# crisprVerse/screenCounter

Measured on AMD Instinct MI355X. Metric: Mreads/s (whole node) + achieved HBM GB/s, 100M x 150bp vs 100k barcodes <=1mm, higher is better.
Workload: dtype u8; 1 GPU; config2: countSingleBarcodes 100000000 reads x 150bp, library 100000, <=1mm, use_first=True; reads_per_gpu=100000000, read_len=150, max_mismatches=1, strand=both, parallelism=read-sharded x1, inputs=resident in HBM, settle_steps=440

## Files before the change

screencounter_amd/csrc/scg_common.h:

```cpp
#ifndef SCG_COMMON_H
#define SCG_COMMON_H

#include <stdint.h>
#include <hip/hip_vector_types.h>

#define SCG_MAX_TEMPLATE 256
#define SCG_MAX_REGIONS 8
#define SCG_COMBO_REGIONS 2
#define SCG_MAX_BARCODE 32
#define SCG_MAX_WIDE_BARCODE 64
#define SCG_MAX_BIG_BARCODE 256
#define SCG_BIG_WORDS 4
#define SCG_MAX_SEGMENTS 6
#define SCG_MAX_SEEDS 4
#define SCG_SEED_LEN 10
#define SCG_EMPTY_KEY (~0ull)
#define SCG_SLOT_EMPTY 0xFFFFFFFEu
#define SCG_HOT_SLOTS 4096

#define SCG_MISSING (-1)
#define SCG_AMBIGUOUS (-2)

#define SCG_SEED_STEPS 16
struct ScgSeedWalk {
    uint32_t w[SCG_SEED_STEPS / 4];
};

struct ScgSeed {
    int32_t len;
    uint32_t nsteps;
    int32_t blk;
    int32_t pad;
    ScgSeedWalk walk[4];
};

struct ScgSeeds {
    int32_t nseeds;
    int32_t pad[3];
    ScgSeed seed[SCG_MAX_SEEDS];
};

struct ScgScan {
    int32_t len;
    int32_t nreg;
    int32_t fstart[SCG_MAX_REGIONS];
    int32_t rstart[SCG_MAX_REGIONS];
    int32_t flen[SCG_MAX_REGIONS];
    int32_t rlen[SCG_MAX_REGIONS];
    ScgSeeds fseeds, rseeds;
    int32_t compact_ok;
    int32_t pad[3];
    uint32_t fplane0[SCG_MAX_TEMPLATE / 32], fplane1[SCG_MAX_TEMPLATE / 32], fmask[SCG_MAX_TEMPLATE / 32];
    uint32_t rplane0[SCG_MAX_TEMPLATE / 32], rplane1[SCG_MAX_TEMPLATE / 32], rmask[SCG_MAX_TEMPLATE / 32];
};

struct ScgTemplate {
    int32_t len;
    int32_t nconst;
    int32_t nreg;
    int32_t fstart[SCG_MAX_REGIONS];
    int32_t rstart[SCG_MAX_REGIONS];
    int32_t flen[SCG_MAX_REGIONS];
    int32_t rlen[SCG_MAX_REGIONS];
    uint8_t fpos[SCG_MAX_TEMPLATE];
    uint8_t fcode[SCG_MAX_TEMPLATE];
    uint8_t rpos[SCG_MAX_TEMPLATE];
    uint8_t rcode[SCG_MAX_TEMPLATE];
};

struct ScgIndex {
    const uint4* nodes;
    const uint4* tables;
    uint32_t slot_mask;
    int32_t n_entries;
    int32_t len;
    int32_t nseg;
    int32_t wide;
    int32_t nwalk[4];
    uint64_t segmask[SCG_MAX_SEGMENTS];
};

struct ScgPairTable {
    const uint64_t* keys;
    const int32_t* vals;
    uint32_t mask;
    int32_t n_entries;
    const uint64_t* list_key1;
    const uint64_t* list_key2;
    const int32_t* list_vals;
};

struct ScgCounters {
    int32_t* base;
    uint32_t replica_mask;
    uint32_t replica_shift;
    int32_t* unit_index;
    uint64_t* unit_pair;
    int32_t* hot;
};

struct ScgReads {
    const uint8_t* seqs;
    const uint32_t* offsets;
    int32_t fixed_len;
    int32_t max_len;
    int32_t ablate;
};

struct ScgSingleParams {
    ScgScan scan;
    const ScgTemplate* tmpl;
    ScgIndex index;
    int32_t max_mm;
    int32_t use_first;
    int32_t fwd, rev;
};

struct ScgComboParams {
    ScgScan scan;
    const ScgTemplate* tmpl;
    ScgIndex index[SCG_COMBO_REGIONS];
    int32_t n_pool[SCG_COMBO_REGIONS];
    int32_t max_mm;
    int32_t use_first;
    int32_t fwd, rev;
    const int32_t* only_if_negative;
    int32_t keep_first;
    int32_t pad;
};

struct ScgDualParams {
    ScgScan scan1, scan2;
    const ScgTemplate* tmpl1;
    const ScgTemplate* tmpl2;
    ScgIndex index1, index2;
    ScgPairTable pairs;
    int32_t rev1, rev2;
    int32_t max_mm1, max_mm2;
    int32_t randomized;
    int32_t use_first;
    int32_t diagnostics;
    int32_t n_pool;
    int32_t n_uid2;
    int32_t keep_first;
    const int32_t* only_if_negative;
    int32_t* overflow;
};

static inline
#ifdef __HIPCC__
__host__ __device__
#endif
uint32_t scg_hash64(uint64_t key) {
    uint32_t h = (uint32_t)key * 0x9E3779B1u;
    h ^= h >> 16;
    h = (h ^ (uint32_t)(key >> 32)) * 0x85EBCA6Bu;
    h ^= h >> 13;
    h *= 0xC2B2AE35u;
    h ^= h >> 16;
    return h;
}

static inline
#ifdef __HIPCC__
__host__ __device__
#endif
uint32_t scg_hash128(uint64_t lo, uint64_t hi) {
    uint32_t a = scg_hash64(lo), b = scg_hash64(hi);
    uint32_t h = (a ^ ((b << 15) | (b >> 17))) * 0x9E3779B1u;
    return h ^ (h >> 15);
}

static inline
#ifdef __HIPCC__
__host__ __device__
#endif
uint32_t scg_hash_big(const uint64_t* lo, const uint64_t* hi) {
    uint32_t h = scg_hash128(lo[0], hi[0]);
    for (int k = 1; k < SCG_BIG_WORDS; ++k) {
        h = (h ^ scg_hash128(lo[k] + k, hi[k])) * 0x85EBCA6Bu;
        h ^= h >> 13;
    }
    return h;
}

static inline
#ifdef __HIPCC__
__host__ __device__
#endif
void scg_big_group(uint64_t ranges, uint64_t mask[SCG_BIG_WORDS]) {
    for (int k = 0; k < SCG_BIG_WORDS; ++k) mask[k] = 0;
    for (int r = 0; r < 2; ++r) {
        const int a = (int)((ranges >> (32 * r)) & 0xFFFFu), b = (int)((ranges >> (32 * r + 16)) & 0xFFFFu);
        for (int k = 0; k < SCG_BIG_WORDS; ++k) {
            const int lo = a > 64 * k ? a : 64 * k, hi = b < 64 * (k + 1) ? b : 64 * (k + 1);
            if (hi <= lo) continue;
            const int n = hi - lo;
            mask[k] |= (n >= 64 ? ~0ull : ((1ull << n) - 1ull)) << (lo - 64 * k);
        }
    }
}

#endif
```

screencounter_amd/csrc/scg_engine.hip.h:

```cpp
#ifndef SCG_ENGINE_HIP_H
#define SCG_ENGINE_HIP_H

#include <hip/hip_runtime.h>
#include "scg_common.h"

namespace scgdev {

__device__ __forceinline__ int base_code(uint32_t c) {
    uint32_t k = (c >> 1) & 3u;
    uint32_t expect = (0x47544341u >> (8u * k)) & 0xFFu;
    return ((c & 0xDFu) == expect) ? (int)k : -1;
}

struct Read {
    const uint8_t* p;
    int n;
};

__device__ __forceinline__ void count_one(const ScgCounters& C, int64_t i) {
    const uint32_t gid = blockIdx.x * blockDim.x + threadIdx.x;
    atomicAdd(C.base + ((i << C.replica_shift) | (int64_t)(gid & C.replica_mask)), 1);
}

__device__ __forceinline__ void count_flagged(const ScgCounters& C, int which, int64_t i, bool flag) {
    const uint64_t m = __ballot(flag);
    if (m == 0) return;
    const int leader = __ffsll((long long)m) - 1;
    if ((int)(threadIdx.x & 63u) == leader) {
        const uint32_t gid = blockIdx.x * blockDim.x + threadIdx.x;
        int32_t* dst = C.hot ? C.hot + which * SCG_HOT_SLOTS + ((gid >> 6) & (SCG_HOT_SLOTS - 1))
                             : C.base + ((i << C.replica_shift) | (int64_t)(gid & C.replica_mask));
        atomicAdd(dst, (int)__popcll(m));
    }
}

__device__ __forceinline__ Read get_read(const ScgReads& R, int64_t i) {
    Read r;
    if (R.offsets) {
        uint32_t a = R.offsets[i], b = R.offsets[i + 1];
        r.p = R.seqs + a;
        r.n = (int)(b - a);
    } else {
        r.p = R.seqs + (size_t)i * (size_t)R.fixed_len;
        r.n = R.fixed_len;
    }
    return r;
}

__device__ __forceinline__ int const_mismatches(const ScgTemplate* __restrict__ T, bool reverse,
                                                const uint8_t* __restrict__ read, int p, int limit) {
    const uint8_t* pos = reverse ? T->rpos : T->fpos;
    const uint8_t* code = reverse ? T->rcode : T->fcode;
    int mm = 0;
    int nconst = T->nconst;
    for (int k = 0; k < nconst; ++k) {
        int c = base_code(read[p + pos[k]]);
        mm += (c != (int)code[k]);
        if (mm > limit) break;
    }
    return mm;
}

struct Big {
    uint64_t w[SCG_BIG_WORDS];
    __device__ __forceinline__ Big() {}
    __device__ __forceinline__ Big(uint64_t x) {
        w[0] = x;
#pragma unroll
        for (int k = 1; k < SCG_BIG_WORDS; ++k) w[k] = 0;
    }
    __device__ __forceinline__ explicit operator bool() const {
        uint64_t any = 0;
#pragma unroll
        for (int k = 0; k < SCG_BIG_WORDS; ++k) any |= w[k];
        return any != 0;
    }
};
#define SCG_BIG_BINARY(OP) \
    __device__ __forceinline__ Big operator OP(const Big& a, const Big& b) { \
        Big r; \
        _Pragma("unroll") for (int k = 0; k < SCG_BIG_WORDS; ++k) r.w[k] = a.w[k] OP b.w[k]; \
        return r; \
    } \
    __device__ __forceinline__ Big& operator OP##=(Big& a, const Big& b) { a = a OP b; return a; }
SCG_BIG_BINARY(&)
SCG_BIG_BINARY(|)
SCG_BIG_BINARY(^)
#undef SCG_BIG_BINARY
__device__ __forceinline__ Big operator~(const Big& a) {
    Big r;
#pragma unroll
    for (int k = 0; k < SCG_BIG_WORDS; ++k) r.w[k] = ~a.w[k];
    return r;
}
__device__ __forceinline__ bool operator==(const Big& a, const Big& b) {
    uint64_t d = 0;
#pragma unroll
    for (int k = 0; k < SCG_BIG_WORDS; ++k) d |= a.w[k] ^ b.w[k];
    return d == 0;
}
__device__ __forceinline__ bool operator!=(const Big& a, const Big& b) { return !(a == b); }
__device__ __forceinline__ Big operator<<(const Big& a, int n) {
    Big r;
    const int q = n >> 6, sh = n & 63;
#pragma unroll
    for (int k = 0; k < SCG_BIG_WORDS; ++k) {
        uint64_t v = 0;
#pragma unroll
        for (int j = 0; j < SCG_BIG_WORDS; ++j) {
            if (j == k - q) v |= a.w[j] << sh;
            if (j == k - q - 1 && sh) v |= a.w[j] >> (64 - sh);
        }
        r.w[k] = v;
    }
    return r;
}
__device__ __forceinline__ Big operator>>(const Big& a, int n) {
    Big r;
    const int q = n >> 6, sh = n & 63;
#pragma unroll
    for (int k = 0; k < SCG_BIG_WORDS; ++k) {
        uint64_t v = 0;
#pragma unroll
        for (int j = 0; j < SCG_BIG_WORDS; ++j) {
            if (j == k + q) v |= a.w[j] >> sh;
            if (j == k + q + 1 && sh) v |= a.w[j] << (64 - sh);
        }
        r.w[k] = v;
    }
    return r;
}

template<class W>
struct QueryT {
    W lo, hi;
    W other;
    int n_other;
};
using Query = QueryT<uint32_t>;

__device__ __forceinline__ uint32_t low_mask(int len) { return len >= 32 ? 0xFFFFFFFFu : ((1u << len) - 1u); }
template<class W> __device__ __forceinline__ W low_mask_w(int len);
template<> __device__ __forceinline__ uint32_t low_mask_w<uint32_t>(int len) { return low_mask(len); }
template<> __device__ __forceinline__ uint64_t low_mask_w<uint64_t>(int len) { return len >= 64 ? ~0ull : ((1ull << len) - 1ull); }

template<> __device__ __forceinline__ Big low_mask_w<Big>(int len) {
    Big r;
#pragma unroll
    for (int k = 0; k < SCG_BIG_WORDS; ++k) {
        const int n = len - 64 * k;
        r.w[k] = n >= 64 ? ~0ull : (n <= 0 ? 0ull : ((1ull << n) - 1ull));
    }
    return r;
}

__device__ __forceinline__ int popcount_w(uint32_t x) { return __popc(x); }
__device__ __forceinline__ int popcount_w(uint64_t x) { return __popcll(x); }
__device__ __forceinline__ uint32_t bitrev_w(uint32_t x) { return __brev(x); }
__device__ __forceinline__ uint64_t bitrev_w(uint64_t x) { return __brevll(x); }
__device__ __forceinline__ int popcount_w(const Big& x) {
    int n = 0;
#pragma unroll
    for (int k = 0; k < SCG_BIG_WORDS; ++k) n += __popcll(x.w[k]);
    return n;
}
__device__ __forceinline__ Big bitrev_w(const Big& x) {
    Big r;
#pragma unroll
    for (int k = 0; k < SCG_BIG_WORDS; ++k) r.w[k] = __brevll(x.w[SCG_BIG_WORDS - 1 - k]);
    return r;
}

template<class W>
__device__ __forceinline__ QueryT<W> reverse_complement(const QueryT<W>& q, int len) {
    QueryT<W> r;
    const int sh = (int)(8 * sizeof(W)) - len;
    const W m = low_mask_w<W>(len);
    r.lo = bitrev_w(q.lo) >> sh;
    r.hi = (~(bitrev_w(q.hi) >> sh)) & m;
    r.other = bitrev_w(q.other) >> sh;
    r.hi &= ~r.other;
    r.n_other = q.n_other;
    return r;
}

template<class W = uint32_t>
__device__ __forceinline__ QueryT<W> pack_region(const uint8_t* __restrict__ s, int len, bool reverse) {
    QueryT<W> q;
    q.lo = 0; q.hi = 0; q.other = 0;
    for (int j = 0; j < len; ++j) {
        int c = base_code(s[j]);
        if (c < 0) {
            q.other |= (W)1 << j;
        } else {
            q.lo |= (W)(c & 1) << j;
            q.hi |= (W)(c >> 1) << j;
        }
    }
    q.n_other = popcount_w(q.other);
    return reverse ? reverse_complement(q, len) : q;
}

template<class W>
__device__ __forceinline__ int query_distance(const QueryT<W>& q, W elo, W ehi, W lenmask) {
    W mism = ((q.lo ^ elo) | (q.hi ^ ehi)) & ~q.other & lenmask;
    return popcount_w(mism) + q.n_other;
}

__device__ __forceinline__ uint4 load_node(const uint4* p) {
    uint4 v = *p;
    asm volatile("" : "+v"(v.x), "+v"(v.y), "+v"(v.z), "+v"(v.w));
    return v;
}

template<class W> struct KeyOps;
template<> struct KeyOps<uint32_t> {
    struct Node { uint32_t lo, hi; int val, next; };
    static constexpr int STRIDE = 1;
    static __device__ __forceinline__ Node load(const uint4* base, size_t i) {
        const uint4 v = load_node(base + i);
        return Node{v.x, v.y, (int)v.z, (int)v.w};
    }
    static __device__ __forceinline__ uint32_t plane_mask(uint64_t m, int plane) { return plane ? (uint32_t)(m >> 32) : (uint32_t)m; }
    static __device__ __forceinline__ uint32_t hash(uint32_t lo, uint32_t hi) { return scg_hash64(((uint64_t)hi << 32) | lo); }
};
template<> struct KeyOps<uint64_t> {
    struct Node { uint64_t lo, hi; int val, next; };
    static constexpr int STRIDE = 2;
    static __device__ __forceinline__ Node load(const uint4* base, size_t i) {
        const uint4 a = load_node(base + 2 * i), b = load_node(base + 2 * i + 1);
        return Node{((uint64_t)a.y << 32) | a.x, ((uint64_t)a.w << 32) | a.z, (int)b.x, (int)b.y};
    }
    static __device__ __forceinline__ uint64_t plane_mask(uint64_t m, int) { return m; }
    static __device__ __forceinline__ uint32_t hash(uint64_t lo, uint64_t hi) { return scg_hash128(lo, hi); }
};
template<> struct KeyOps<Big> {
    struct Node { Big lo, hi; int val, next; };
    static constexpr int STRIDE = 5;
    static __device__ __forceinline__ Node load(const uint4* base, size_t i) {
        Node n;
        const uint4* p = base + 5 * i;
#pragma unroll
        for (int k = 0; k < 2; ++k) {
            const uint4 a = load_node(p + k), b = load_node(p + 2 + k);
            n.lo.w[2 * k] = ((uint64_t)a.y << 32) | a.x; n.lo.w[2 * k + 1] = ((uint64_t)a.w << 32) | a.z;
            n.hi.w[2 * k] = ((uint64_t)b.y << 32) | b.x; n.hi.w[2 * k + 1] = ((uint64_t)b.w << 32) | b.z;
        }
        const uint4 c = load_node(p + 4);
        n.val = (int)c.x; n.next = (int)c.y;
        return n;
    }
    static __device__ __forceinline__ Big plane_mask(uint64_t ranges, int) {
        Big m;
        scg_big_group(ranges, m.w);
        return m;
    }
    static __device__ __forceinline__ uint32_t hash(const Big& lo, const Big& hi) { return scg_hash_big(lo.w, hi.w); }
};

template<class W, class F>
__device__ __forceinline__ void index_search(const ScgIndex& X, const QueryT<W>& q, int cap, F f,
                                             const int* best = nullptr) {
    typedef KeyOps<W> K;
    if (q.n_other > cap) return;
    const W lm = low_mask_w<W>(X.len);
    if (X.nseg == 0) {
        for (int e = 0; e < X.n_entries; ++e) {
            const typename K::Node ent = K::load(X.nodes, (size_t)e);
            int d = query_distance<W>(q, ent.lo, ent.hi, lm);
            if (d <= cap && f(ent.val, d)) return;
        }
        return;
    }
    const int w0 = __builtin_amdgcn_readfirstlane(X.nwalk[0]), w1 = __builtin_amdgcn_readfirstlane(X.nwalk[1]);
    const int w2 = __builtin_amdgcn_readfirstlane(X.nwalk[2]), w3 = __builtin_amdgcn_readfirstlane(X.nwalk[3]);
    auto tables_for = [&](int c) { return c <= 0 ? w0 : (c == 1 ? w1 : (c == 2 ? w2 : w3)); };
    int nwalk = tables_for(cap);
    const uint32_t nslots = X.slot_mask + 1u;
#pragma unroll 1
    for (int s = 0; s < nwalk; ++s) {
        const uint64_t mask = X.segmask[s];
        const W mlo = K::plane_mask(mask, 0), mhi = K::plane_mask(mask, 1);
        if (q.other & mlo) continue;
        const W sklo = q.lo & mlo, skhi = q.hi & mhi;
        uint32_t pos = K::hash(sklo, skhi) & X.slot_mask;
        const uint4* table = X.tables + (size_t)s * nslots * K::STRIDE;
        typename K::Node ent;
        bool found = false;
        for (;;) {
            ent = K::load(table, (size_t)pos);
            if ((uint32_t)ent.next == SCG_SLOT_EMPTY) break;
            if ((ent.lo & mlo) == sklo && (ent.hi & mhi) == skhi) { found = true; break; }
            pos = (pos + 1) & X.slot_mask;
        }
        if (!found) continue;
        const uint4* nodes = X.nodes + (size_t)s * (size_t)X.n_entries * K::STRIDE;
        for (;;) {
            int d = query_distance<W>(q, ent.lo, ent.hi, lm);
            if (d <= cap && f(ent.val, d)) return;
            const int e = ent.next;
            if (e < 0) break;
            ent = K::load(nodes, (size_t)e);
        }
        if (best && *best < cap) {
            const int t = tables_for(*best);
            nwalk = t < nwalk ? t : nwalk;
        }
    }
}

template<class W>
__device__ __forceinline__ void index_match(const ScgIndex& X, const QueryT<W>& q, int cap, int& index, int& mm,
                                            bool keep_first = false) {
    int best = cap + 1, cur = SCG_MISSING;
    index_search<W>(X, q, cap, [&](int v, int d) -> bool {
        if (d < best) { best = d; cur = v; }
        else if (d == best && cur != v) { cur = keep_first ? (v < cur ? v : cur) : SCG_AMBIGUOUS; }
        return d == 0;
    }, &best);
    index = cur; mm = best;
}

__device__ __forceinline__ int pair_probe(const ScgPairTable& t, int u1, int u2) {
    uint64_t key = ((uint64_t)(uint32_t)u1 << 32) | (uint32_t)u2;
    uint32_t h = scg_hash64(key) & t.mask;
    for (;;) {
        uint64_t k = t.keys[h];
        if (k == key) return t.vals[h];
        if (k == SCG_EMPTY_KEY) return -1;
        h = (h + 1) & t.mask;
    }
}

template<int K, class W>
__device__ __forceinline__ bool index_neighbours(const ScgIndex& X, const QueryT<W>& q, int cap, int val[K], int dist[K], int& n) {
    n = 0;
    bool overflow = false;
    index_search<W>(X, q, cap, [&](int v, int d) -> bool {
        bool seen = false;
#pragma unroll
        for (int i = 0; i < K; ++i) seen |= (i < n && val[i] == v);
        if (!seen) {
            if (n == K) { overflow = true; return true; }
#pragma unroll
            for (int i = 0; i < K; ++i) {
                if (i == n) { val[i] = v; dist[i] = d; }
            }
            ++n;
        }
        return false;
    });
    return !overflow;
}

template<class W>
__device__ __forceinline__ void pair_match(const ScgIndex& X1, const ScgIndex& X2, const ScgPairTable& P,
                                           const QueryT<W>& q1, int cap1, const QueryT<W>& q2, int cap2,
                                           int& index, int& total) {
    index = SCG_MISSING; total = 0;
    if (q1.n_other > cap1 || q2.n_other > cap2) return;
    int best = cap1 + cap2 + 1, cur = SCG_MISSING;
    auto consider = [&](int u1, int d1, int u2, int d2) {
        int tot = d1 + d2;
        if (tot > best) return;
        int v = pair_probe(P, u1, u2);
        if (v >= 0) {
            if (tot < best) { best = tot; cur = v; }
            else if (cur != v) { cur = SCG_AMBIGUOUS; }
        }
    };
    if (sizeof(W) >= 8 || (X1.nseg != 0 && X2.nseg != 0)) {
#ifndef SCG_PAIR_K
#define SCG_PAIR_K 4
#endif
        constexpr int K = SCG_PAIR_K;
        int v1[K], d1[K], n1, v2[K], d2[K], n2;
        const bool ok1 = index_neighbours<K, W>(X1, q1, cap1, v1, d1, n1);
        if (ok1 && n1 == 0) return;
        const bool ok2 = index_neighbours<K, W>(X2, q2, cap2, v2, d2, n2);
        if (ok2 && n2 == 0) return;
        if (ok1 && ok2) {
#pragma unroll
            for (int i = 0; i < K; ++i) {
#pragma unroll
                for (int j = 0; j < K; ++j) {
                    if (i < n1 && j < n2) consider(v1[i], d1[i], v2[j], d2[j]);
                }
            }
        } else {
            index_search<W>(X1, q1, cap1, [&](int u1, int e1) -> bool {
                index_search<W>(X2, q2, cap2, [&](int u2, int e2) -> bool {
                    consider(u1, e1, u2, e2);
                    return false;
                });
                return false;
            });
        }
    } else if constexpr (sizeof(W) == 4) {
        uint32_t lm1 = low_mask(X1.len), lm2 = low_mask(X2.len);
        for (int i = 0; i < P.n_entries; ++i) {
            uint64_t k1 = P.list_key1[i];
            int e1 = query_distance<uint32_t>(q1, (uint32_t)k1, (uint32_t)(k1 >> 32), lm1);
            if (e1 > cap1) continue;
            uint64_t k2 = P.list_key2[i];
            int e2 = query_distance<uint32_t>(q2, (uint32_t)k2, (uint32_t)(k2 >> 32), lm2);
            if (e2 > cap2) continue;
            int tot = e1 + e2, v = P.list_vals[i];
            if (tot < best) { best = tot; cur = v; }
            else if (tot == best && cur != v) { cur = SCG_AMBIGUOUS; }
        }
    }
    if (cur != SCG_MISSING) { index = cur; total = best; }
}

}

#endif
```

screencounter_amd/csrc/scg_kernels.hip:

```cpp
#include <hip/hip_runtime.h>

#include <cmath>
#include <cstdlib>
#include <mutex>

#include "scg_engine.hip.h"
#include "scg_staged.hip.h"
#include "scg_launch.h"

using namespace scgdev;

namespace {

constexpr int BLOCK = 256;

#ifndef SCG_SINGLE_WAVES
#define SCG_SINGLE_WAVES 8
#endif
#ifndef SCG_COMBO_WAVES
#define SCG_COMBO_WAVES 8
#endif

template<class W>
__device__ __forceinline__ QueryT<W> pack_regions(const ScgTemplate* T, const uint8_t* __restrict__ window, bool reverse, int total_len) {
    QueryT<W> q;
    q.lo = 0; q.hi = 0; q.other = 0;
    int off = 0;
    for (int r = 0; r < T->nreg; ++r) {
        const int start = reverse ? T->rstart[r] : T->fstart[r], len = reverse ? T->rlen[r] : T->flen[r];
        for (int j = 0; j < len; ++j) {
            int c = base_code(window[start + j]);
            if (c < 0) {
                q.other |= (W)1 << (off + j);
            } else {
                q.lo |= (W)(c & 1) << (off + j);
                q.hi |= (W)(c >> 1) << (off + j);
            }
        }
        off += len;
    }
    q.n_other = popcount_w(q.other);
    return reverse ? reverse_complement(q, total_len) : q;
}

template<class W = uint32_t>
__device__ __forceinline__ int single_read(const ScgSingleParams& P, const Read& rd) {
    const ScgTemplate* T = P.tmpl;
    const int len = T->len;
    const int max_mm = P.max_mm;
    int found = 0, index = -1, best = max_mm + 1;
    for (int p = 0; p + len <= rd.n; ++p) {
        for (int s = 0; s < 2; ++s) {
            if (s == 0 ? !P.fwd : !P.rev) continue;
            int c = const_mismatches(T, s != 0, rd.p, p, max_mm);
            if (c > max_mm) continue;
            QueryT<W> q = pack_regions<W>(T, rd.p + p, s != 0, P.index.len);
            int idx, d;
            index_match<W>(P.index, q, max_mm - c, idx, d);
            if (idx < 0) continue;
            int tot = c + d;
            if (P.use_first) {
                return idx;
            } else if (tot == best) {
                if (index != idx) { found = 0; index = -1; }
            } else if (tot < best) {
                found = 1; best = tot; index = idx;
            }
        }
    }
    return found ? index : -1;
}

template<class W>
__global__ __launch_bounds__(BLOCK) void single_kernel(ScgSingleParams P, ScgReads R, int64_t n_reads,
                                                        ScgCounters counts) {
    int64_t i = (int64_t)blockIdx.x * BLOCK + threadIdx.x;
    if (i >= n_reads) return;
    Read rd = get_read(R, i);
    int idx = single_read<W>(P, rd);
    if (counts.unit_index) counts.unit_index[i] = idx;
    else if (idx >= 0) count_one(counts, idx);
}

struct BestHit {
    int best, code;
    bool tied;
    __device__ __forceinline__ void offer(int c, int p, bool reverse) {
        if (c < best) { best = c; code = (p << 1) | (reverse ? 1 : 0); tied = false; }
        else if (c == best) { tied = true; }
    }
};

__global__ __launch_bounds__(BLOCK) void random_kernel(ScgSingleParams P, ScgReads R, int64_t n_reads, int32_t* __restrict__ hits) {
    int64_t i = (int64_t)blockIdx.x * BLOCK + threadIdx.x;
    if (i >= n_reads) return;
    Read rd = get_read(R, i);
    const ScgTemplate* T = P.tmpl;
    BestHit h{P.max_mm + 1, -1, false};
    int out = -1;
    for (int p = 0; p + T->len <= rd.n && out < 0; ++p) {
        for (int s = 0; s < 2; ++s) {
            if (s == 0 ? !P.fwd : !P.rev) continue;
            int c = const_mismatches(T, s != 0, rd.p, p, P.max_mm);
            if (c > P.max_mm) continue;
            if (P.use_first) { out = (p << 1) | s; break; }
            h.offer(c, p, s != 0);
        }
    }
    if (!P.use_first && !h.tied && h.best <= P.max_mm) out = h.code;
    hits[i] = out;
}

template<class W>
__device__ __forceinline__ bool combo_candidate(const ScgComboParams& P, const Read& rd, int p, bool reverse, int c,
                                                int out[SCG_COMBO_REGIONS], int& total) {
    const ScgTemplate* T = P.tmpl;
    int obs = c;
    for (int r = 0; r < SCG_COMBO_REGIONS; ++r) {
        int slot = reverse ? (SCG_COMBO_REGIONS - 1 - r) : r;
        int start = reverse ? T->rstart[r] : T->fstart[r];
        const ScgIndex& tab = P.index[slot];
        QueryT<W> q = pack_region<W>(rd.p + p + start, tab.len, reverse);
        int idx, d;
        index_match<W>(tab, q, P.max_mm - obs, idx, d, P.keep_first != 0);
        if (idx < 0) return false;
        obs += d;
        if (obs > P.max_mm) return false;
        out[slot] = idx;
    }
    total = obs;
    return true;
}

template<class W>
__device__ __forceinline__ int combo_read(const ScgComboParams& P, const Read& rd, int best_id[SCG_COMBO_REGIONS]) {
    const ScgTemplate* T = P.tmpl;
    const int len = T->len;
    int found = 0, best = P.max_mm + 1;
    for (int p = 0; p + len <= rd.n && !(found && P.use_first); ++p) {
        for (int s = 0; s < 2; ++s) {
            if (s == 0 ? !P.fwd : !P.rev) continue;
            int c = const_mismatches(T, s != 0, rd.p, p, P.max_mm);
            if (c > P.max_mm) continue;
            int cand[SCG_COMBO_REGIONS], tot;
            if (!combo_candidate<W>(P, rd, p, s != 0, c, cand, tot)) continue;
            if (P.use_first) {
                found = 1; best_id[0] = cand[0]; best_id[1] = cand[1];
                break;
            } else if (tot <= best) {
                if (tot == best) {
                    if (best_id[0] != cand[0] || best_id[1] != cand[1]) found = 0;
                } else {
                    found = 1; best = tot; best_id[0] = cand[0]; best_id[1] = cand[1];
                }
            }
        }
    }
    return found;
}

template<class W>
__global__ __launch_bounds__(BLOCK) void combo_kernel(ScgComboParams P, ScgReads R, int64_t n_reads,
                                                       ScgCounters cells) {
    int64_t i = (int64_t)blockIdx.x * BLOCK + threadIdx.x;
    if (i >= n_reads) return;
    if (P.only_if_negative && P.only_if_negative[i] >= 0) return;
    Read rd = get_read(R, i);
    int best_id[SCG_COMBO_REGIONS] = {0, 0};
    const bool found = combo_read<W>(P, rd, best_id) != 0;
    if (cells.unit_pair) cells.unit_pair[i] = found ? (((uint64_t)(uint32_t)best_id[0] << 32) | (uint32_t)best_id[1]) : ~0ull;
    else if (found) count_one(cells, (int64_t)best_id[0] * P.n_pool[1] + best_id[1]);
}

template<class W>
__device__ __forceinline__ int dual_first(const ScgDualParams& P, const Read& a, const Read& b) {
    const ScgTemplate* T1 = P.tmpl1;
    const ScgTemplate* T2 = P.tmpl2;
    int s1 = P.rev1 ? T1->rstart[0] : T1->fstart[0];
    int s2 = P.rev2 ? T2->rstart[0] : T2->fstart[0];
    for (int p1 = 0; p1 + T1->len <= a.n; ++p1) {
        int c1 = const_mismatches(T1, P.rev1 != 0, a.p, p1, P.max_mm1);
        if (c1 > P.max_mm1) continue;
        QueryT<W> q1 = pack_region<W>(a.p + p1 + s1, P.index1.len, P.rev1 != 0);
        for (int p2 = 0; p2 + T2->len <= b.n; ++p2) {
            int c2 = const_mismatches(T2, P.rev2 != 0, b.p, p2, P.max_mm2);
            if (c2 > P.max_mm2) continue;
            QueryT<W> q2 = pack_region<W>(b.p + p2 + s2, P.index2.len, P.rev2 != 0);
            int idx, tot;
            pair_match<W>(P.index1, P.index2, P.pairs, q1, P.max_mm1 - c1, q2, P.max_mm2 - c2, idx, tot);
            if (idx >= 0) return idx;
        }
    }
    return -1;
}

template<class W>
__device__ __forceinline__ void dual_best(const ScgDualParams& P, const Read& a, const Read& b, int& chosen, int& best) {
    const ScgTemplate* T1 = P.tmpl1;
    const ScgTemplate* T2 = P.tmpl2;
    int s1 = P.rev1 ? T1->rstart[0] : T1->fstart[0];
    int s2 = P.rev2 ? T2->rstart[0] : T2->fstart[0];
    chosen = -1;
    best = P.max_mm1 + P.max_mm2 + 1;
    for (int p1 = 0; p1 + T1->len <= a.n; ++p1) {
        int c1 = const_mismatches(T1, P.rev1 != 0, a.p, p1, P.max_mm1);
        if (c1 > P.max_mm1) continue;
        QueryT<W> q1 = pack_region<W>(a.p + p1 + s1, P.index1.len, P.rev1 != 0);
        for (int p2 = 0; p2 + T2->len <= b.n; ++p2) {
            int c2 = const_mismatches(T2, P.rev2 != 0, b.p, p2, P.max_mm2);
            if (c2 > P.max_mm2) continue;
            QueryT<W> q2 = pack_region<W>(b.p + p2 + s2, P.index2.len, P.rev2 != 0);
            int idx, tot;
            pair_match<W>(P.index1, P.index2, P.pairs, q1, P.max_mm1 - c1, q2, P.max_mm2 - c2, idx, tot);
            if (idx >= 0) {
                int cur = tot + c1 + c2;
                if (cur < best) { chosen = idx; best = cur; }
                else if (cur == best && chosen != idx) { chosen = -1; }
            }
        }
    }
}

template<class W>
__device__ __forceinline__ bool mate_search(const ScgTemplate* T, const ScgIndex& X, bool reverse, int max_mm, bool use_first,
                                            bool keep_first, const Read& rd, int& index, int& mism) {
    bool found = false;
    index = -1; mism = 0;
    int best = max_mm + 1;
    const int start = reverse ? T->rstart[0] : T->fstart[0];
    for (int p = 0; p + T->len <= rd.n; ++p) {
        int c = const_mismatches(T, reverse, rd.p, p, max_mm);
        if (c > max_mm) continue;
        QueryT<W> q = pack_region<W>(rd.p + p + start, X.len, reverse);
        int idx, d;
        index_match<W>(X, q, max_mm - c, idx, d, keep_first);
        if (idx < 0) continue;
        int tot = c + d;
        if (use_first) { index = idx; mism = tot; return true; }
        if (tot == best) {
            if (index != idx) { found = false; index = -1; }
        } else if (tot < best) {
            found = true; best = tot; index = idx; mism = tot;
        }
    }
    return found;
}

template<class M>
__device__ __forceinline__ void diagnose_pair(const ScgDualParams& P, const M& m, const ScgCounters& counters) {
    const int64_t b1_only = P.n_pool, b2_only = b1_only + 1, cells = b2_only + 1;
    auto emit = [&](int u1, int u2) {
        if (counters.unit_pair) counters.unit_pair[(int64_t)blockIdx.x * blockDim.x + threadIdx.x] = ((uint64_t)(uint32_t)u1 << 32) | (uint32_t)u2;
        else count_one(counters, cells + (int64_t)u1 * P.n_uid2 + u2);
    };
    int i1 = -1, m1 = 0, i2 = -1, m2 = 0, j1 = -1, n1 = 0, j2 = -1, n2 = 0;
    const bool f1 = m.search1(P, 0, i1, m1);
    const bool f2 = m.search2(P, 1, i2, m2);
    const bool swapped = P.randomized && !(P.use_first && f1 && f2);
    bool g1 = false, g2 = false;
    if (swapped) {
        g1 = m.search1(P, 1, j1, n1);
        g2 = m.search2(P, 0, j2, n2);
    }
    int what = 0, u1 = 0, u2 = 0;
    auto pick = [&](int x, int y) { what = 1; u1 = x; u2 = y; };
    if (P.use_first) {
        if (f1 && f2) pick(i1, i2);
        else if (P.randomized) {
            if (g1 && g2) pick(j1, j2);
            else if (f1 || g1) what = 2;
            else if (f2 || g2) what = 3;
        } else {
            if (f1) what = 2;
            else if (f2) what = 3;
        }
    } else if (!P.randomized) {
        if (f1 && f2) pick(i1, i2);
        else if (f1) what = 2;
        else if (f2) what = 3;
    } else if (f1 && f2) {
        if (g1 && g2) {
            int mism = m1 + m2, rmism = n1 + n2;
            if (mism > rmism) pick(j1, j2);
            else if (mism < rmism) pick(i1, i2);
            else if (i1 == j1 && i2 == j2) pick(i1, i2);
        } else {
            pick(i1, i2);
        }
    } else {
        if (g1 && g2) pick(j1, j2);
        else if (f1 || g1) what = 2;
        else if (f2 || g2) what = 3;
    }
    if (what == 1) emit(u1, u2);
    count_flagged(counters, 0, b1_only, what == 2);
    count_flagged(counters, 1, b2_only, what == 3);
}

template<class W>
__device__ __forceinline__ int dual_pair(const ScgDualParams& P, const Read& a, const Read& b) {
    int idx;
    if (P.use_first) {
        idx = dual_first<W>(P, a, b);
        if (idx < 0 && P.randomized) idx = dual_first<W>(P, b, a);
    } else {
        int best;
        dual_best<W>(P, a, b, idx, best);
        if (P.randomized) {
            int idx2, best2;
            dual_best<W>(P, b, a, idx2, best2);
            if (idx < 0 || best > best2) { idx = idx2; best = best2; }
            else if (best == best2 && idx != idx2) { idx = -1; }
        }
    }
    return idx;
}

template<class W>
struct GeneralMates {
    Read a, b;
    __device__ __forceinline__ bool search1(const ScgDualParams& P, int which, int& index, int& mism) const {
        return mate_search<W>(P.tmpl1, P.index1, P.rev1 != 0, P.max_mm1, P.use_first != 0, P.keep_first != 0, which ? b : a, index, mism);
    }
    __device__ __forceinline__ bool search2(const ScgDualParams& P, int which, int& index, int& mism) const {
        return mate_search<W>(P.tmpl2, P.index2, P.rev2 != 0, P.max_mm2, P.use_first != 0, P.keep_first != 0, which ? b : a, index, mism);
    }
};

template<class W>
__global__ __launch_bounds__(BLOCK) void dual_kernel(ScgDualParams P, ScgReads R1, ScgReads R2, int64_t n_pairs,
                                                      ScgCounters counts) {
    int64_t i = (int64_t)blockIdx.x * BLOCK + threadIdx.x;
    if (i >= n_pairs) return;
    if (P.diagnostics == 2 && P.only_if_negative && P.only_if_negative[i] >= 0) return;
    Read a = get_read(R1, i), b = get_read(R2, i);
    int idx = P.diagnostics == 2 ? -1 : dual_pair<W>(P, a, b);
    if (idx >= 0) {
        count_one(counts, idx);
    } else if (P.diagnostics) {
        diagnose_pair(P, GeneralMates<W>{a, b}, counts);
    }
}

template<int NW, int NT, int NC, class W>
__device__ __forceinline__ int single_read_staged(const ScgSingleParams& P, const Tile<NW>& tile, const StrandTable<NT>& st, const StagedRead& sr, int ablate = 0) {
    const ScgScan& T = P.scan;
    const int max_mm = P.max_mm;
    uint32_t candF[NC], candR[NC];
    scan_read<NW, NC>(tile, sr, T, P.fwd != 0, P.rev != 0, candF, candR);
#ifdef SCG_ABLATE
    if (ablate == 1) return (candF[0] ^ candR[NC - 1]) == 0x12345u ? 0 : -1;
#endif
    int found = 0, index = -1, best = max_mm + 1;
    const int last = last_position(sr.n, T.len);
    for (;;) {
        int pf = first_bit<NC>(candF), pr = first_bit<NC>(candR);
        bool rev = pr < pf;
        int p = rev ? pr : pf;
        if (p > last) break;
        clear_bit<NC>(candF, rev ? -1 : p);
        clear_bit<NC>(candR, rev ? p : -1);
        int c = window_mismatches<NW, NT>(tile, sr.bit + p, st, rev);
        if (c > max_mm) continue;
        QueryT<W> q;
        if constexpr (sizeof(W) == 4) {
            const int start = region_start<NT>(st, 0, rev);
            q = region_query<NW>(tile, sr.bit + p + start, P.index.len, rev);
        } else {
            q = regions_query<NW, NT, W>(tile, sr.bit + p, st, uniform(T.nreg), P.index.len, rev);
        }
        int idx, d;
        index_match<W>(P.index, q, max_mm - c, idx, d);
        if (idx < 0) continue;
        int tot = c + d;
        if (P.use_first) {
            return idx;
        } else if (tot == best) {
            if (index != idx) { found = 0; index = -1; }
        } else if (tot < best) {
            found = 1; best = tot; index = idx;
        }
    }
    return found ? index : -1;
}

template<int NW, int NT, int NC, class W>
__global__ __launch_bounds__(STAGE_BLOCK, SCG_SINGLE_WAVES) __attribute__((amdgpu_num_sgpr(80))) void single_staged_kernel(ScgSingleParams P, ScgReads R, int64_t n_reads,
                                                                   ScgCounters counts, int32_t* __restrict__ error_flag) {
    __shared__ Tile<NW> tile;
    __shared__ StrandTable<NT> strands;
    fill_strand_table<NT>(strands, P.scan);
    const int64_t r0 = (int64_t)blockIdx.x * STAGE_BLOCK;
    const int nr = (int)((n_reads - r0) < STAGE_BLOCK ? (n_reads - r0) : STAGE_BLOCK);
    int64_t span0 = 0;
    const bool staged = (P.scan.len <= 32 * NT) && stage_reads<NW>(R, n_reads, r0, nr, tile, span0);
    __syncthreads();
    if ((int)threadIdx.x >= nr) return;
    Read rd = get_read(R, r0 + threadIdx.x);
    if (!staged || rd.n > 32 * NW) {
        *error_flag = 1;
        return;
    }
    StagedRead sr;
    sr.bit = (int)((int64_t)(rd.p - R.seqs) - span0);
    sr.n = rd.n;
    int idx;
#ifdef SCG_ABLATE
    if (R.ablate == 2) {
        idx = (tile.p0[threadIdx.x] == 0xdeadbeefu) ? 0 : -1;
    } else {
        idx = single_read_staged<NW, NT, NC, W>(P, tile, strands, sr, R.ablate);
    }
    if (R.ablate == 3 && idx != 0x7ffffff0 && !counts.unit_index) return;
#else
    idx = single_read_staged<NW, NT, NC, W>(P, tile, strands, sr);
#endif
    if (counts.unit_index) counts.unit_index[r0 + threadIdx.x] = idx;
    else if (idx >= 0) count_one(counts, idx);
}

template<int NW, int NT, int NC>
__global__ __launch_bounds__(STAGE_BLOCK) __attribute__((amdgpu_num_sgpr(80))) void random_staged_kernel(ScgSingleParams P, ScgReads R, int64_t n_reads,
                                                                   int32_t* __restrict__ hits, int32_t* __restrict__ error_flag) {
    __shared__ Tile<NW> tile;
    __shared__ StrandTable<NT> strands;
    fill_strand_table<NT>(strands, P.scan);
    const int64_t r0 = (int64_t)blockIdx.x * STAGE_BLOCK;
    const int nr = (int)((n_reads - r0) < STAGE_BLOCK ? (n_reads - r0) : STAGE_BLOCK);
    int64_t span0 = 0;
    const bool staged = (P.scan.len <= 32 * NT) && stage_reads<NW>(R, n_reads, r0, nr, tile, span0);
    __syncthreads();
    if ((int)threadIdx.x >= nr) return;
    Read rd = get_read(R, r0 + threadIdx.x);
    if (!staged || rd.n > 32 * NW) {
        *error_flag = 1;
        return;
    }
    StagedRead sr;
    sr.bit = (int)((int64_t)(rd.p - R.seqs) - span0);
    sr.n = rd.n;
    uint32_t candF[NC], candR[NC];
    scan_read<NW, NC>(tile, sr, P.scan, P.fwd != 0, P.rev != 0, candF, candR);
    BestHit h{P.max_mm + 1, -1, false};
    int out = -1;
    const int last = last_position(sr.n, P.scan.len);
    for (;;) {
        int pf = first_bit<NC>(candF), pr = first_bit<NC>(candR);
        bool rev = pr < pf;
        int p = rev ? pr : pf;
        if (p > last) break;
        clear_bit<NC>(candF, rev ? -1 : p);
        clear_bit<NC>(candR, rev ? p : -1);
        int c = window_mismatches<NW, NT>(tile, sr.bit + p, strands, rev);
        if (c > P.max_mm) continue;
        if (P.use_first) { out = (p << 1) | (rev ? 1 : 0); break; }
        h.offer(c, p, rev);
    }
    if (!P.use_first && !h.tied && h.best <= P.max_mm) out = h.code;
    hits[r0 + threadIdx.x] = out;
}

template<int NW, int NT, bool SECOND, class W>
__device__ __forceinline__ bool combo_candidate_staged(const ScgComboParams& P, const ScgIndex* pools, const Tile<NW>& tile, const StrandTable<NT>& st, const StagedRead& sr,
                                                       int p, bool reverse, int c, int out[SCG_COMBO_REGIONS], int& total) {
    int obs = c;
#pragma unroll
    for (int r = 0; r < SCG_COMBO_REGIONS; ++r) {
        int slot = reverse ? (SCG_COMBO_REGIONS - 1 - r) : r;
        const int start = region_start<NT>(st, r, reverse);
        const ScgIndex& tab = pools[slot];
        QueryT<W> q = region_query<NW, W>(tile, sr.bit + p + start, tab.len, reverse);
        int idx, d;
        index_match<W>(tab, q, P.max_mm - obs, idx, d, SECOND);
        if (idx < 0) return false;
        obs += d;
        if (obs > P.max_mm) return false;
        out[slot] = idx;
    }
    total = obs;
    return true;
}

template<int NW, int NT, int NC, bool SECOND, class W>
__global__ __launch_bounds__(STAGE_BLOCK, SCG_COMBO_WAVES) __attribute__((amdgpu_num_sgpr(80))) void combo_staged_kernel(ScgComboParams P, ScgReads R, int64_t n_reads,
                                                                  ScgCounters cells, int32_t* __restrict__ error_flag) {
    __shared__ Tile<NW> tile;
    __shared__ StrandTable<NT> strands;
    __shared__ ScgIndex pools[SCG_COMBO_REGIONS];
    fill_strand_table<NT>(strands, P.scan);
    if (threadIdx.x < SCG_COMBO_REGIONS * (sizeof(ScgIndex) / 4)) {
        static_assert(sizeof(ScgIndex) % 4 == 0, "copied by dwords");
        const uint32_t* src = reinterpret_cast<const uint32_t*>(&P.index[0]);
        reinterpret_cast<uint32_t*>(&pools[0])[threadIdx.x] = src[threadIdx.x];
    }
    const int64_t r0 = (int64_t)blockIdx.x * STAGE_BLOCK;
    const int nr = (int)((n_reads - r0) < STAGE_BLOCK ? (n_reads - r0) : STAGE_BLOCK);
    int64_t span0 = 0;
    const bool staged = (P.scan.len <= 32 * NT) && stage_reads<NW>(R, n_reads, r0, nr, tile, span0);
    __syncthreads();
    if ((int)threadIdx.x >= nr) return;
    Read rd = get_read(R, r0 + threadIdx.x);
    int found = 0, best = P.max_mm + 1;
    int best_id[SCG_COMBO_REGIONS] = {0, 0};
    if (!staged || rd.n > 32 * NW) {
        *error_flag = 1;
        return;
    }
    if (!(SECOND && P.only_if_negative[r0 + threadIdx.x] >= 0)) {
        const ScgScan& T = P.scan;
        StagedRead sr;
        sr.bit = (int)((int64_t)(rd.p - R.seqs) - span0);
        sr.n = rd.n;
        uint32_t candF[NC], candR[NC];
        scan_read<NW, NC>(tile, sr, T, P.fwd != 0, P.rev != 0, candF, candR);
        const int last = last_position(sr.n, T.len);
        for (;;) {
            int pf = first_bit<NC>(candF), pr = first_bit<NC>(candR);
            bool rev = pr < pf;
            int p = rev ? pr : pf;
            if (p > last) break;
            clear_bit<NC>(candF, rev ? -1 : p);
            clear_bit<NC>(candR, rev ? p : -1);
            int c = window_mismatches<NW, NT>(tile, sr.bit + p, strands, rev);
            if (c > P.max_mm) continue;
            int cand[SCG_COMBO_REGIONS], tot;
            if (!combo_candidate_staged<NW, NT, SECOND, W>(P, pools, tile, strands, sr, p, rev, c, cand, tot)) continue;
            if (P.use_first) {
                found = 1; best_id[0] = cand[0]; best_id[1] = cand[1];
                break;
            } else if (tot <= best) {
                if (tot == best) {
                    if (best_id[0] != cand[0] || best_id[1] != cand[1]) found = 0;
                } else {
                    found = 1; best = tot; best_id[0] = cand[0]; best_id[1] = cand[1];
                }
            }
        }
    }
    if (cells.unit_index) cells.unit_index[r0 + threadIdx.x] = found ? best_id[0] * P.n_pool[1] + best_id[1] : -1;
    else if (cells.unit_pair) cells.unit_pair[r0 + threadIdx.x] = found ? (((uint64_t)(uint32_t)best_id[0] << 32) | (uint32_t)best_id[1]) : ~0ull;
    else if (found) count_one(cells, (int64_t)best_id[0] * P.n_pool[1] + best_id[1]);
}

template<int NW, int NT, int NC, class W>
__device__ __forceinline__ bool mate_search_staged(const Tile<NW>& tile, const StagedRead& sr, const ScgScan& T, const ScgIndex& X,
                                                   bool reverse, int max_mm, bool use_first, bool keep_first, int& index, int& mism) {
    bool found = false;
    index = -1; mism = 0;
    int best = max_mm + 1;
    uint32_t cand[NC], unused[NC];
    scan_read<NW, NC>(tile, sr, T, true, false, cand, unused);
    const int start = T.fstart[0];
    const int last = last_position(sr.n, T.len);
    for (;;) {
        int p = first_bit<NC>(cand);
        if (p > last) break;
        clear_bit<NC>(cand, p);
        int c = window_mismatches<NW, NT>(tile, sr.bit + p, T, false);
        if (c > max_mm) continue;
        QueryT<W> q = region_query<NW, W>(tile, sr.bit + p + start, X.len, reverse);
        int idx, d;
        index_match<W>(X, q, max_mm - c, idx, d, keep_first);
        if (idx < 0) continue;
        int tot = c + d;
        if (use_first) { index = idx; mism = tot; return true; }
        if (tot == best) {
            if (index != idx) { found = false; index = -1; }
        } else if (tot < best) {
            found = true; best = tot; index = idx; mism = tot;
        }
    }
    return found;
}

template<int NW, int NT, int NC, class W>
__device__ __forceinline__ void dual_orientation_staged(const ScgDualParams& P, const bool BEST,
                                                        const Tile<NW>& ta, const StagedRead& a,
                                                        const Tile<NW>& tb, const StagedRead& b,
                                                        int& chosen, int& best) {
    const ScgScan& T1 = P.scan1;
    const ScgScan& T2 = P.scan2;
    const bool rev1 = P.rev1 != 0, rev2 = P.rev2 != 0;
    const int s1 = T1.fstart[0];
    const int s2 = T2.fstart[0];
    chosen = -1;
    best = P.max_mm1 + P.max_mm2 + 1;
    uint32_t c1[NC], c2[NC], unused[NC];
    scan_read<NW, NC>(ta, a, T1, true, false, c1, unused);
    scan_read<NW, NC>(tb, b, T2, true, false, c2, unused);
    const int last1 = last_position(a.n, T1.len), last2 = last_position(b.n, T2.len);
    for (;;) {
        int p1 = first_bit<NC>(c1);
        if (p1 > last1) break;
        clear_bit<NC>(c1, p1);
        int m1 = window_mismatches<NW, NT>(ta, a.bit + p1, T1, false);
        if (m1 > P.max_mm1) continue;
        QueryT<W> q1 = region_query<NW, W>(ta, a.bit + p1 + s1, P.index1.len, rev1);
        uint32_t w2[NC];
#pragma unroll
        for (int i = 0; i < NC; ++i) w2[i] = c2[i];
        for (;;) {
            int p2 = first_bit<NC>(w2);
            if (p2 > last2) break;
            clear_bit<NC>(w2, p2);
            int m2 = window_mismatches<NW, NT>(tb, b.bit + p2, T2, false);
            if (m2 > P.max_mm2) {
                clear_bit<NC>(c2, p2);
                continue;
            }
            QueryT<W> q2 = region_query<NW, W>(tb, b.bit + p2 + s2, P.index2.len, rev2);
            int idx, tot;
            pair_match<W>(P.index1, P.index2, P.pairs, q1, P.max_mm1 - m1, q2, P.max_mm2 - m2, idx, tot);
            if (idx >= 0) {
                if (!BEST) { chosen = idx; return; }
                int cur = tot + m1 + m2;
                if (cur < best) { chosen = idx; best = cur; }
                else if (cur == best && chosen != idx) { chosen = -1; }
            }
        }
    }
}

template<class W>
struct MateHits {
    QueryT<W> q;
    int m;
    int count;
};

template<int NW, int NT, int NC, class W>
__device__ __forceinline__ void collect_hits(const Tile<NW>& tile, const StagedRead& sr, const ScgScan& T, int key_len, bool reverse,
                                             int max_mm, MateHits<W>& h) {
    uint32_t cand[NC], unused[NC];
    scan_read<NW, NC>(tile, sr, T, true, false, cand, unused);
    const int last = last_position(sr.n, T.len);
    h.count = 0; h.m = 0;
    h.q = QueryT<W>{};
    for (;;) {
        int p = first_bit<NC>(cand);
        if (p > last) break;
        clear_bit<NC>(cand, p);
        int m = window_mismatches<NW, NT>(tile, sr.bit + p, T, false);
        if (m > max_mm) continue;
        if (h.count == 0) {
            h.q = region_query<NW, W>(tile, sr.bit + p + T.fstart[0], key_len, reverse);
            h.m = m;
        }
        ++h.count;
    }
}

template<class W>
__device__ __forceinline__ void dual_orientation_hits(const ScgDualParams& P, const bool BEST, const MateHits<W>& x, const MateHits<W>& y,
                                                      int& chosen, int& best) {
    chosen = -1;
    best = P.max_mm1 + P.max_mm2 + 1;
    if (x.count == 0 || y.count == 0) return;
    int idx, tot;
    pair_match<W>(P.index1, P.index2, P.pairs, x.q, P.max_mm1 - x.m, y.q, P.max_mm2 - y.m, idx, tot);
    if (idx >= 0) { chosen = idx; best = tot + x.m + y.m; }
}

struct SearchedMates {
    int index[4], mism[4];
    bool found[4];
    __device__ __forceinline__ bool search1(const ScgDualParams&, int which, int& i, int& m) const { i = index[2 * which]; m = mism[2 * which]; return found[2 * which]; }
    __device__ __forceinline__ bool search2(const ScgDualParams&, int which, int& i, int& m) const { i = index[2 * which + 1]; m = mism[2 * which + 1]; return found[2 * which + 1]; }
};

template<class W>
struct PairState {
    MateHits<W> h1a, h2a, h1b, h2b;
    SearchedMates sm;
    bool bad;
};

template<int NW, int NT, int NC, bool MATES_ONLY, bool RANDOMIZED, class W>
__device__ __forceinline__ void dual_pass(const int pass, const ScgDualParams& P, const ScgReads& R1, const ScgReads& R2, int64_t n_pairs,
                                          int64_t r0, int nr, bool fits, bool wanted, Tile<NW>& tile, PairState<W>& S) {
    ScgReads R;
    R.seqs = pass ? R2.seqs : R1.seqs; R.offsets = pass ? R2.offsets : R1.offsets;
    R.fixed_len = pass ? R2.fixed_len : R1.fixed_len; R.max_len = pass ? R2.max_len : R1.max_len;
    int64_t span = 0;
    if (pass) __syncthreads();
    const bool ok = fits && stage_reads<NW>(R, n_pairs, r0, nr, tile, span);
    __syncthreads();
    S.bad = S.bad || !ok;
    if (!ok || !wanted) return;
    Read rd = get_read(R, r0 + threadIdx.x);
    if (rd.n > 32 * NW) { S.bad = true; return; }
    StagedRead sr;
    sr.bit = (int)((int64_t)(rd.p - R.seqs) - span); sr.n = rd.n;
    bool do1 = pass == 0 || RANDOMIZED, do2 = pass == 1 || RANDOMIZED;
    if (MATES_ONLY) {
        SearchedMates& sm = S.sm;
        if (RANDOMIZED && pass == 1 && P.use_first && sm.found[0]) {
            int i2, m2;
            const bool f2 = mate_search_staged<NW, NT, NC, W>(tile, sr, P.scan2, P.index2, P.rev2 != 0, P.max_mm2, P.use_first != 0, P.keep_first != 0, i2, m2);
            sm.found[3] = f2; sm.index[3] = i2; sm.mism[3] = m2;
            do2 = false;
            do1 = !f2;
        }
        int i1 = -1, m1 = 0, i2 = -1, m2 = 0;
        bool f1 = false, f2 = false;
        if (do1) f1 = mate_search_staged<NW, NT, NC, W>(tile, sr, P.scan1, P.index1, P.rev1 != 0, P.max_mm1, P.use_first != 0, P.keep_first != 0, i1, m1);
        if (do2) f2 = mate_search_staged<NW, NT, NC, W>(tile, sr, P.scan2, P.index2, P.rev2 != 0, P.max_mm2, P.use_first != 0, P.keep_first != 0, i2, m2);
        if (pass == 0) { sm.found[0] = f1; sm.index[0] = i1; sm.mism[0] = m1; sm.found[1] = f2; sm.index[1] = i2; sm.mism[1] = m2; }
        else {
            sm.found[2] = f1; sm.index[2] = i1; sm.mism[2] = m1;
            if (do2) { sm.found[3] = f2; sm.index[3] = i2; sm.mism[3] = m2; }
        }
    } else {
        MateHits<W> t1, t2;
        t1.count = t2.count = 0; t1.m = t2.m = 0;
        t1.q = t2.q = QueryT<W>{};
        if (do1) collect_hits<NW, NT, NC, W>(tile, sr, P.scan1, P.index1.len, P.rev1 != 0, P.max_mm1, t1);
        if (do2) collect_hits<NW, NT, NC, W>(tile, sr, P.scan2, P.index2.len, P.rev2 != 0, P.max_mm2, t2);
        if (pass == 0) { S.h1a = t1; S.h2a = t2; } else { S.h1b = t1; S.h2b = t2; }
    }
}

template<int NW, int NT, int NC, bool MATES_ONLY, bool RANDOMIZED, class W>
__global__ __launch_bounds__(STAGE_BLOCK) void dual_passes_kernel(ScgDualParams P, ScgReads R1, ScgReads R2, int64_t n_pairs,
                                                                 ScgCounters counts, int32_t* __restrict__ error_flag) {
    __shared__ Tile<NW> tile;
    const int64_t r0 = (int64_t)blockIdx.x * STAGE_BLOCK;
    const int nr = (int)((n_pairs - r0) < STAGE_BLOCK ? (n_pairs - r0) : STAGE_BLOCK);
    const bool fits = P.scan1.len <= 32 * NT && P.scan2.len <= 32 * NT;
    const bool lane = (int)threadIdx.x < nr;
    const bool wanted = lane && !(MATES_ONLY && P.only_if_negative && P.only_if_negative[r0 + threadIdx.x] >= 0);
    PairState<W> S;
    S.bad = !fits;
    S.h1a.count = S.h2a.count = S.h1b.count = S.h2b.count = 0;
    S.h1a.m = S.h2a.m = S.h1b.m = S.h2b.m = 0;
    S.h1a.q = S.h2a.q = S.h1b.q = S.h2b.q = QueryT<W>{};
#pragma unroll
    for (int k = 0; k < 4; ++k) { S.sm.index[k] = -1; S.sm.mism[k] = 0; S.sm.found[k] = false; }

    if (RANDOMIZED) {
#pragma unroll 1
        for (int pass = 0; pass < 2; ++pass) dual_pass<NW, NT, NC, MATES_ONLY, RANDOMIZED, W>(pass, P, R1, R2, n_pairs, r0, nr, fits, wanted, tile, S);
    } else {
        dual_pass<NW, NT, NC, MATES_ONLY, RANDOMIZED, W>(0, P, R1, R2, n_pairs, r0, nr, fits, wanted, tile, S);
        dual_pass<NW, NT, NC, MATES_ONLY, RANDOMIZED, W>(1, P, R1, R2, n_pairs, r0, nr, fits, wanted, tile, S);
    }
    if (!lane) return;
    if (S.bad) { *error_flag = 1; return; }
    if (!wanted) return;
    if (MATES_ONLY) {
        diagnose_pair(P, S.sm, counts);
        return;
    }
    int idx = -1;
    if (S.h1a.count > 1 || S.h2b.count > 1 || S.h1b.count > 1 || S.h2a.count > 1) {
        const int slot = atomicAdd(P.overflow, 1);
        P.overflow[1 + slot] = (int32_t)(r0 + threadIdx.x);
        if (counts.unit_index) counts.unit_index[r0 + threadIdx.x] = -1;
        return;
    }
    const bool best_mode = !P.use_first;
    int best;
    dual_orientation_hits<W>(P, best_mode, S.h1a, S.h2b, idx, best);
    if (RANDOMIZED && (best_mode || idx < 0)) {
        int ci, cb;
        dual_orientation_hits<W>(P, best_mode, S.h1b, S.h2a, ci, cb);
        if (!best_mode) idx = ci;
        else if (idx < 0 || best > cb) { idx = ci; best = cb; }
        else if (best == cb && idx != ci) { idx = -1; }
    }
    if (counts.unit_index) counts.unit_index[r0 + threadIdx.x] = idx;
    else if (idx >= 0) count_one(counts, idx);
}

template<class W>
__global__ __launch_bounds__(BLOCK) void dual_overflow_kernel(ScgDualParams P, ScgReads R1, ScgReads R2, ScgCounters counts) {
    const int n = P.overflow[0];
    for (int k = blockIdx.x * BLOCK + threadIdx.x; k < n; k += gridDim.x * BLOCK) {
        const int64_t i = P.overflow[1 + k];
        Read a = get_read(R1, i), b = get_read(R2, i);
        const int idx = dual_pair<W>(P, a, b);
        if (counts.unit_index) counts.unit_index[i] = idx;
        else if (idx >= 0) count_one(counts, idx);
    }
}

template<int NW, int NT, int NC, class W>
__global__ __launch_bounds__(STAGE_BLOCK) void dual_staged_kernel(ScgDualParams P, ScgReads R1, ScgReads R2, int64_t n_pairs,
                                                                 ScgCounters counts, int32_t* __restrict__ error_flag) {
    __shared__ Tile<NW> tile1;
    __shared__ Tile<NW> tile2;
    const int64_t r0 = (int64_t)blockIdx.x * STAGE_BLOCK;
    const int nr = (int)((n_pairs - r0) < STAGE_BLOCK ? (n_pairs - r0) : STAGE_BLOCK);
    int64_t span1 = 0, span2 = 0;
    const bool fits = P.scan1.len <= 32 * NT && P.scan2.len <= 32 * NT;
    const bool ok1 = fits && stage_reads<NW>(R1, n_pairs, r0, nr, tile1, span1);
    const bool ok2 = ok1 && stage_reads<NW>(R2, n_pairs, r0, nr, tile2, span2);
    __syncthreads();
    if ((int)threadIdx.x >= nr) return;
    Read a = get_read(R1, r0 + threadIdx.x), b = get_read(R2, r0 + threadIdx.x);
    if (!ok2 || a.n > 32 * NW || b.n > 32 * NW) {
        *error_flag = 1;
        return;
    }
    StagedRead sa, sb;
    sa.bit = (int)((int64_t)(a.p - R1.seqs) - span1); sa.n = a.n;
    sb.bit = (int)((int64_t)(b.p - R2.seqs) - span2); sb.n = b.n;
    const bool best_mode = !P.use_first;
    const int norient = P.randomized ? 2 : 1;
    int best = 0, idx = -1;
    for (int o = 0; o < norient; ++o) {
        const Tile<NW>* ta = o ? &tile2 : &tile1;
        const Tile<NW>* tb = o ? &tile1 : &tile2;
        const StagedRead ra = o ? sb : sa, rb = o ? sa : sb;
        int ci, cb;
        dual_orientation_staged<NW, NT, NC, W>(P, best_mode, *ta, ra, *tb, rb, ci, cb);
        if (!best_mode) {
            idx = ci;
            if (ci >= 0) break;
        } else if (o == 0) {
            idx = ci; best = cb;
        } else {
            if (idx < 0 || best > cb) { idx = ci; best = cb; }
            else if (best == cb && idx != ci) { idx = -1; }
        }
    }
    if (counts.unit_index) counts.unit_index[r0 + threadIdx.x] = idx;
    else if (idx >= 0) count_one(counts, idx);
}

template<class W>
__global__ __launch_bounds__(BLOCK) void match_kernel(ScgIndex tab, const uint8_t* __restrict__ seqs, int32_t n, int cap, int reverse,
                                                       int32_t* __restrict__ index_out, int32_t* __restrict__ mm_out) {
    int i = blockIdx.x * BLOCK + threadIdx.x;
    if (i >= n) return;
    QueryT<W> q = pack_region<W>(seqs + (size_t)i * tab.len, tab.len, reverse != 0);
    int idx, d;
    index_match<W>(tab, q, cap, idx, d);
    index_out[i] = idx >= 0 ? idx : -1;
    mm_out[i] = idx >= 0 ? d : -1;
}

__device__ __forceinline__ uint64_t splitmix64(uint64_t& s) {
    uint64_t z = (s += 0x9E3779B97F4A7C15ull);
    z = (z ^ (z >> 30)) * 0xBF58476D1CE4E5B9ull;
    z = (z ^ (z >> 27)) * 0x94D049BB133111EBull;
    return z ^ (z >> 31);
}
__device__ __forceinline__ float u01(uint64_t& s) { return (float)(splitmix64(s) >> 40) * (1.0f / 16777216.0f); }
__device__ __forceinline__ uint32_t below(uint64_t& s, uint32_t n) { return (uint32_t)(((splitmix64(s) >> 32) * (uint64_t)n) >> 32); }

__global__ __launch_bounds__(BLOCK) void synth_kernel(scg_synth_spec S, char* __restrict__ out, int64_t n_reads) {
    int64_t i = (int64_t)blockIdx.x * BLOCK + threadIdx.x;
    if (i >= n_reads) return;
    const char B[4] = {'A', 'C', 'G', 'T'};
    uint64_t g = (uint64_t)(S.first_read + i);
    uint64_t shared = S.seed ^ (g * 0xD1342543DE82EF95ull);
    uint64_t priv = (S.seed + 0x632BE59BD9B4E019ull * (uint64_t)(S.pair_column + 1)) ^ (g * 0xA0761D6478BD642Full);
    char* dst = out + (size_t)i * (size_t)S.read_len;
    const int L = S.read_len, T = S.template_len;

    bool junk = u01(shared) < S.p_junk || T > L;
    bool flip = u01(shared) < S.p_reverse;
    int k0 = 0, k1 = 0;
    if (S.d_pair_index) {
        bool invalid = u01(shared) < S.p_invalid_pair;
        uint32_t row = below(shared, (uint32_t)S.n_pairs);
        uint32_t row2 = below(shared, (uint32_t)S.n_pairs);
        int r = (invalid && S.pair_column == 1) ? (int)row2 : (int)row;
        k0 = S.d_pair_index[2 * (size_t)r + S.pair_column];
    } else {
        k0 = (int)below(shared, (uint32_t)(S.n_pool[0] > 0 ? S.n_pool[0] : 1));
        k1 = (int)below(shared, (uint32_t)(S.n_pool[1] > 0 ? S.n_pool[1] : 1));
    }
    int offset = junk ? 0 : (int)below(shared, (uint32_t)(L - T + 1));

    for (int j = 0; j < L; ++j) {
        char c = B[below(priv, 4)];
        if (!junk && j >= offset && j < offset + T) {
            int t = j - offset;
            char tc = S.d_template[t];
            if (tc != '-') {
                c = tc;
            } else {
                for (int r = 0; r < S.n_regions; ++r) {
                    int rel = t - S.region_start[r];
                    if (rel >= 0 && rel < S.region_len[r]) {
                        int k = r == 0 ? k0 : k1;
                        c = S.d_pool[r][(size_t)k * S.region_len[r] + rel];
                    }
                }
            }
            if (u01(priv) < S.p_sub) {
                uint32_t cur = c == 'A' ? 0 : c == 'C' ? 1 : c == 'G' ? 2 : 3;
                c = B[(cur + 1 + below(priv, 3)) & 3];
            }
        }
        if (u01(priv) < S.p_n) c = 'N';
        dst[j] = c;
    }
    if (flip) {
        for (int a = 0, b = L - 1; a <= b; ++a, --b) {
            char x = dst[a], y = dst[b];
            auto comp = [](char ch) { return ch == 'A' ? 'T' : ch == 'C' ? 'G' : ch == 'G' ? 'C' : ch == 'T' ? 'A' : ch; };
            dst[a] = comp(y);
            dst[b] = comp(x);
        }
    }
}

inline size_t extra_lds() {
    static const size_t kb = [] { const char* e = std::getenv("SCG_EXTRA_LDS_KB"); return e ? (size_t)std::atoi(e) : (size_t)0; }();
    return kb << 10;
}
inline unsigned grid_for(int64_t n) { return (unsigned)((n + BLOCK - 1) / BLOCK); }
inline unsigned staged_grid(int64_t n) { return (unsigned)((n + STAGE_BLOCK - 1) / STAGE_BLOCK); }

}

namespace scg {

bool force_general() {
    const char* e = std::getenv("SCG_FORCE_GENERAL");
    return e && *e && *e != '0';
}

namespace {

template<template<int, int> class Launch, class... Args>
hipError_t dispatch_shape(int max_len, int tmpl_len, Args&&... args) {
    const bool wide = max_len > 160;
    if (tmpl_len <= 64) return wide ? Launch<10, 2>::go(args...) : Launch<5, 2>::go(args...);
    if (tmpl_len <= 128) return wide ? Launch<10, 4>::go(args...) : Launch<5, 4>::go(args...);
    return wide ? Launch<10, 8>::go(args...) : Launch<5, 8>::go(args...);
}

template<int NW, int NT> struct LaunchSingle {
    static hipError_t go(const ScgSingleParams& P, const ScgReads& R, int64_t n, const ScgCounters& counts, int32_t* flag, hipStream_t stream) {
        const bool compact = NW == 5 && P.scan.compact_ok && R.max_len - P.scan.len + 1 <= 96;
        if (P.index.wide || P.scan.nreg != 1) {
            if (compact) hipLaunchKernelGGL((single_staged_kernel<NW, NT, (NW == 5 ? 3 : NW), uint64_t>), dim3(staged_grid(n)), dim3(STAGE_BLOCK), extra_lds(), stream, P, R, n, counts, flag);
            else hipLaunchKernelGGL((single_staged_kernel<NW, NT, NW, uint64_t>), dim3(staged_grid(n)), dim3(STAGE_BLOCK), extra_lds(), stream, P, R, n, counts, flag);
        } else if (compact) {
            hipLaunchKernelGGL((single_staged_kernel<NW, NT, (NW == 5 ? 3 : NW), uint32_t>), dim3(staged_grid(n)), dim3(STAGE_BLOCK), extra_lds(), stream, P, R, n, counts, flag);
        } else {
            hipLaunchKernelGGL((single_staged_kernel<NW, NT, NW, uint32_t>), dim3(staged_grid(n)), dim3(STAGE_BLOCK), extra_lds(), stream, P, R, n, counts, flag);
        }
        return hipGetLastError();
    }
};
template<int NW, int NT> struct LaunchCombo {
    template<int NC, class W>
    static void run(const ScgComboParams& P, const ScgReads& R, int64_t n, const ScgCounters& cells, int32_t* flag, hipStream_t stream) {
        if (P.only_if_negative) hipLaunchKernelGGL((combo_staged_kernel<NW, NT, NC, true, W>), dim3(staged_grid(n)), dim3(STAGE_BLOCK), extra_lds(), stream, P, R, n, cells, flag);
        else hipLaunchKernelGGL((combo_staged_kernel<NW, NT, NC, false, W>), dim3(staged_grid(n)), dim3(STAGE_BLOCK), extra_lds(), stream, P, R, n, cells, flag);
    }
    static hipError_t go(const ScgComboParams& P, const ScgReads& R, int64_t n, const ScgCounters& cells, int32_t* flag, hipStream_t stream) {
        const bool compact = NW == 5 && P.scan.compact_ok && R.max_len - P.scan.len + 1 <= 96;
        constexpr int NCC = NW == 5 ? 3 : NW;
        const bool wide = P.index[0].wide != 0;
        if (compact) { if (wide) run<NCC, uint64_t>(P, R, n, cells, flag, stream); else run<NCC, uint32_t>(P, R, n, cells, flag, stream); }
        else { if (wide) run<NW, uint64_t>(P, R, n, cells, flag, stream); else run<NW, uint32_t>(P, R, n, cells, flag, stream); }
        return hipGetLastError();
    }
};
static double expected_chance_hits(const ScgScan& T, int max_mm, int read_len) {
    int c = 0;
    for (int w = 0; w < SCG_MAX_TEMPLATE / 32; ++w) c += __builtin_popcount(T.fmask[w]);
    double ways = 0, choose = 1, pow3 = 1;
    for (int k = 0; k <= max_mm && k <= c; ++k) {
        ways += choose * pow3;
        choose = choose * (c - k) / (k + 1);
        pow3 *= 3;
    }
    return (double)(read_len > T.len ? read_len - T.len + 1 : 1) * ways / std::pow(4.0, c);
}

static int two_tiles() {
    static const int v = [] { const char* e = getenv("SCG_DUAL_TWO_TILES"); return e && *e ? atoi(e) : -1; }();
    return v;
}

template<int NW, int NT> struct LaunchDual {
    template<int NC, class W>
    static void run(const ScgDualParams& P, const ScgReads& R1, const ScgReads& R2, int64_t n, const ScgCounters& counts, int32_t* flag, hipStream_t stream, bool passes) {
        if (P.diagnostics) {
            if (P.randomized) hipLaunchKernelGGL((dual_passes_kernel<NW, NT, NC, true, true, W>), dim3(staged_grid(n)), dim3(STAGE_BLOCK), extra_lds(), stream, P, R1, R2, n, counts, flag);
            else hipLaunchKernelGGL((dual_passes_kernel<NW, NT, NC, true, false, W>), dim3(staged_grid(n)), dim3(STAGE_BLOCK), extra_lds(), stream, P, R1, R2, n, counts, flag);
        } else if (passes) {
            (void)hipMemsetAsync(P.overflow, 0, sizeof(int32_t), stream);
            if (P.randomized) hipLaunchKernelGGL((dual_passes_kernel<NW, NT, NC, false, true, W>), dim3(staged_grid(n)), dim3(STAGE_BLOCK), extra_lds(), stream, P, R1, R2, n, counts, flag);
            else hipLaunchKernelGGL((dual_passes_kernel<NW, NT, NC, false, false, W>), dim3(staged_grid(n)), dim3(STAGE_BLOCK), extra_lds(), stream, P, R1, R2, n, counts, flag);
            hipLaunchKernelGGL((dual_overflow_kernel<W>), dim3(256), dim3(BLOCK), 0, stream, P, R1, R2, counts);
        } else {
            hipLaunchKernelGGL((dual_staged_kernel<NW, NT, NC, W>), dim3(staged_grid(n)), dim3(STAGE_BLOCK), extra_lds(), stream, P, R1, R2, n, counts, flag);
        }
    }
    static hipError_t go(const ScgDualParams& P, const ScgReads& R1, const ScgReads& R2, int64_t n, const ScgCounters& counts, int32_t* flag, hipStream_t stream) {
        const int max_len = R1.max_len > R2.max_len ? R1.max_len : R2.max_len;
        const int min_t = P.scan1.len < P.scan2.len ? P.scan1.len : P.scan2.len;
        const bool compact = NW == 5 && P.scan1.compact_ok && P.scan2.compact_ok && max_len - min_t + 1 <= 96;
        constexpr int NCC = NW == 5 ? 3 : NW;
        if (P.diagnostics == 1) return hipErrorInvalidValue;
        const bool wide = P.index1.wide != 0;
        const int forced = two_tiles();
        const bool passes = P.overflow && (forced >= 0 ? forced == 0
                                           : expected_chance_hits(P.scan1, P.max_mm1, max_len) + expected_chance_hits(P.scan2, P.max_mm2, max_len) < 0.01);
        if (compact) { if (wide) run<NCC, uint64_t>(P, R1, R2, n, counts, flag, stream, passes); else run<NCC, uint32_t>(P, R1, R2, n, counts, flag, stream, passes); }
        else { if (wide) run<NW, uint64_t>(P, R1, R2, n, counts, flag, stream, passes); else run<NW, uint32_t>(P, R1, R2, n, counts, flag, stream, passes); }
        return hipGetLastError();
    }
};

}

static bool use_general(int max_len) { return force_general() || max_len <= 0 || max_len > 320; }

hipError_t launch_single(const ScgSingleParams& P, int tmpl_len, const ScgReads& R, int64_t n, const ScgCounters& counts, int32_t* flag, hipStream_t stream) {
    if (n <= 0) return hipSuccess;
    if (use_general(R.max_len) || P.index.wide == 2) {
        if (P.index.wide == 2) hipLaunchKernelGGL(single_kernel<Big>, dim3(grid_for(n)), dim3(BLOCK), 0, stream, P, R, n, counts);
        else if (P.index.wide || P.scan.nreg != 1) hipLaunchKernelGGL(single_kernel<uint64_t>, dim3(grid_for(n)), dim3(BLOCK), 0, stream, P, R, n, counts);
        else hipLaunchKernelGGL(single_kernel<uint32_t>, dim3(grid_for(n)), dim3(BLOCK), 0, stream, P, R, n, counts);
        return hipGetLastError();
    }
    return dispatch_shape<LaunchSingle>(R.max_len, tmpl_len, P, R, n, counts, flag, stream);
}

template<int NW, int NT> struct LaunchRandom {
    static hipError_t go(const ScgSingleParams& P, const ScgReads& R, int64_t n, int32_t* hits, int32_t* flag, hipStream_t stream) {
        if (NW == 5 && P.scan.compact_ok && R.max_len - P.scan.len + 1 <= 96) {
            hipLaunchKernelGGL((random_staged_kernel<NW, NT, (NW == 5 ? 3 : NW)>), dim3(staged_grid(n)), dim3(STAGE_BLOCK), extra_lds(), stream, P, R, n, hits, flag);
        } else {
            hipLaunchKernelGGL((random_staged_kernel<NW, NT, NW>), dim3(staged_grid(n)), dim3(STAGE_BLOCK), extra_lds(), stream, P, R, n, hits, flag);
        }
        return hipGetLastError();
    }
};

hipError_t launch_random(const ScgSingleParams& P, int tmpl_len, const ScgReads& R, int64_t n, int32_t* d_hits, int32_t* flag, hipStream_t stream) {
    if (n <= 0) return hipSuccess;
    if (use_general(R.max_len)) {
        hipLaunchKernelGGL(random_kernel, dim3(grid_for(n)), dim3(BLOCK), 0, stream, P, R, n, d_hits);
        return hipGetLastError();
    }
    return dispatch_shape<LaunchRandom>(R.max_len, tmpl_len, P, R, n, d_hits, flag, stream);
}

hipError_t launch_combo(const ScgComboParams& P, int tmpl_len, const ScgReads& R, int64_t n, const ScgCounters& cells, int32_t* flag, hipStream_t stream) {
    if (n <= 0) return hipSuccess;
    if (use_general(R.max_len) || P.index[0].wide == 2) {
        if (P.index[0].wide == 2) hipLaunchKernelGGL(combo_kernel<Big>, dim3(grid_for(n)), dim3(BLOCK), 0, stream, P, R, n, cells);
        else if (P.index[0].wide) hipLaunchKernelGGL(combo_kernel<uint64_t>, dim3(grid_for(n)), dim3(BLOCK), 0, stream, P, R, n, cells);
        else hipLaunchKernelGGL(combo_kernel<uint32_t>, dim3(grid_for(n)), dim3(BLOCK), 0, stream, P, R, n, cells);
        return hipGetLastError();
    }
    return dispatch_shape<LaunchCombo>(R.max_len, tmpl_len, P, R, n, cells, flag, stream);
}

hipError_t launch_dual(const ScgDualParams& P, int tmpl_len, const ScgReads& R1, const ScgReads& R2, int64_t n, const ScgCounters& counts, int32_t* flag, hipStream_t stream) {
    if (n <= 0) return hipSuccess;
    const int lo_len = R1.max_len < R2.max_len ? R1.max_len : R2.max_len;
    if (use_general(lo_len) || use_general(R1.max_len > R2.max_len ? R1.max_len : R2.max_len) || P.index1.wide == 2) {
        if (P.index1.wide == 2) hipLaunchKernelGGL(dual_kernel<Big>, dim3(grid_for(n)), dim3(BLOCK), 0, stream, P, R1, R2, n, counts);
        else if (P.index1.wide) hipLaunchKernelGGL(dual_kernel<uint64_t>, dim3(grid_for(n)), dim3(BLOCK), 0, stream, P, R1, R2, n, counts);
        else hipLaunchKernelGGL(dual_kernel<uint32_t>, dim3(grid_for(n)), dim3(BLOCK), 0, stream, P, R1, R2, n, counts);
        return hipGetLastError();
    }
    const int max_len = R1.max_len > R2.max_len ? R1.max_len : R2.max_len;
    return dispatch_shape<LaunchDual>(max_len, tmpl_len, P, R1, R2, n, counts, flag, stream);
}

constexpr int TALLY_BLOCK = 1024;

__global__ __launch_bounds__(TALLY_BLOCK) void tally_kernel(const int32_t* __restrict__ unit_index, int64_t n, int32_t* __restrict__ counters,
                                                            int64_t n_counters, int bins) {
    extern __shared__ uint32_t tally_bins[];
    const int64_t lo = (int64_t)blockIdx.y * bins;
    const int nb = (int)((n_counters - lo) < bins ? (n_counters - lo) : bins);
    for (int i = threadIdx.x; i < (bins + 1) / 2; i += TALLY_BLOCK) tally_bins[i] = 0;
    __syncthreads();
    const int64_t quads = (n + 3) / 4;
    const int64_t q0 = quads * blockIdx.x / gridDim.x, q1 = quads * (blockIdx.x + 1) / gridDim.x;
    auto add = [&](int32_t v) {
        const uint32_t b = (uint32_t)(v - (int32_t)lo);
        if (b >= (uint32_t)nb) return;
        const uint32_t sh = (b & 1u) * 16u;
        const uint32_t old = atomicAdd(&tally_bins[b >> 1], 1u << sh);
        if (((old >> sh) & 0xFFFFu) == 0x7FFFu) {
            atomicSub(&tally_bins[b >> 1], 0x8000u << sh);
            atomicAdd(&counters[lo + b], 0x8000);
        }
    };
    typedef int32_t i32x4 __attribute__((ext_vector_type(4)));
    const i32x4* quad = reinterpret_cast<const i32x4*>(unit_index);
    const int64_t q_full = n / 4;
    constexpr int U = 4;
    int64_t q = q0 + threadIdx.x;
    for (; q + (U - 1) * TALLY_BLOCK < q1 && q + (U - 1) * TALLY_BLOCK < q_full; q += U * TALLY_BLOCK) {
        i32x4 v[U];
#pragma unroll
        for (int k = 0; k < U; ++k) v[k] = __builtin_nontemporal_load(quad + q + k * TALLY_BLOCK);
#pragma unroll
        for (int k = 0; k < U; ++k) { add(v[k].x); add(v[k].y); add(v[k].z); add(v[k].w); }
    }
    for (; q < q1; q += TALLY_BLOCK) {
        if (q < q_full) {
            const i32x4 v = __builtin_nontemporal_load(quad + q);
            add(v.x); add(v.y); add(v.z); add(v.w);
        } else {
            for (int64_t i = 4 * q; i < n; ++i) add(unit_index[i]);
        }
    }
    __syncthreads();
    for (int b = threadIdx.x; b < nb; b += TALLY_BLOCK) {
        const uint32_t c = (tally_bins[b >> 1] >> ((b & 1) * 16)) & 0xFFFFu;
        if (c) atomicAdd(&counters[lo + b], (int32_t)c);
    }
}

__global__ __launch_bounds__(BLOCK) void hot_fold_kernel(int32_t* __restrict__ hot, int32_t* __restrict__ pair_of_counters) {
    __shared__ int sums[2][BLOCK / 64];
    for (int which = 0; which < 2; ++which) {
        int acc = 0;
        for (int i = threadIdx.x; i < SCG_HOT_SLOTS; i += BLOCK) {
            int32_t* p = hot + which * SCG_HOT_SLOTS + i;
            if (__hip_atomic_load(p, __ATOMIC_RELAXED, __HIP_MEMORY_SCOPE_AGENT)) acc += atomicExch(p, 0);
        }
        for (int off = 32; off > 0; off >>= 1) acc += __shfl_down(acc, off);
        if ((threadIdx.x & 63) == 0) sums[which][threadIdx.x >> 6] = acc;
    }
    __syncthreads();
    if (threadIdx.x < 2) {
        int tot = 0;
        for (int w = 0; w < BLOCK / 64; ++w) tot += sums[threadIdx.x][w];
        if (tot) atomicAdd(&pair_of_counters[threadIdx.x], tot);
    }
}

__global__ __launch_bounds__(BLOCK) void fold_kernel(int32_t* __restrict__ replicas, int shift, int64_t n,
                                                     int32_t* __restrict__ counters) {
    const int R = 1 << shift;
    if (R < 64) {
        int64_t i = (int64_t)blockIdx.x * BLOCK + threadIdx.x;
        if (i >= n) return;
        int32_t* p = replicas + (i << shift);
        int32_t sum = 0;
        for (int r = 0; r < R; ++r) {
            if (__hip_atomic_load(p + r, __ATOMIC_RELAXED, __HIP_MEMORY_SCOPE_AGENT)) sum += atomicExch(p + r, 0);
        }
        if (sum) atomicAdd(&counters[i], sum);
    } else {
        int64_t i = ((int64_t)blockIdx.x * BLOCK + threadIdx.x) >> 6;
        if (i >= n) return;
        const int lane = threadIdx.x & 63;
        int32_t* p = replicas + (i << shift);
        int32_t sum = 0;
        for (int r = lane; r < R; r += 64) {
            if (__hip_atomic_load(p + r, __ATOMIC_RELAXED, __HIP_MEMORY_SCOPE_AGENT)) sum += atomicExch(p + r, 0);
        }
        for (int off = 32; off > 0; off >>= 1) sum += __shfl_down(sum, off, 64);
        if (lane == 0 && sum) atomicAdd(&counters[i], sum);
    }
}

hipError_t launch_hot_fold(int32_t* hot, int32_t* pair_of_counters, hipStream_t stream) {
    hipLaunchKernelGGL(hot_fold_kernel, dim3(1), dim3(BLOCK), 0, stream, hot, pair_of_counters);
    return hipGetLastError();
}

hipError_t launch_tally(const int32_t* unit_index, int64_t n, int32_t* counters, int64_t n_counters, hipStream_t stream) {
    if (n <= 0 || n_counters <= 0) return hipSuccess;
    const int max_bins = 80 * 1024;
    const int passes = (int)((n_counters + max_bins - 1) / max_bins);
    int bins = (int)((n_counters + passes - 1) / passes);
    bins = (bins + 1) & ~1;
    constexpr int MAX_DEVICES = 64;
    static std::once_flag once[MAX_DEVICES];
    static int cu_count[MAX_DEVICES];
    static hipError_t setup[MAX_DEVICES];
    int dev = 0;
    if (hipGetDevice(&dev) != hipSuccess || dev < 0 || dev >= MAX_DEVICES) return hipErrorInvalidDevice;
    std::call_once(once[dev], [dev] {
        setup[dev] = hipFuncSetAttribute(reinterpret_cast<const void*>(tally_kernel), hipFuncAttributeMaxDynamicSharedMemorySize, 80 * 1024 * 2);
        hipDeviceProp_t prop;
        cu_count[dev] = hipGetDeviceProperties(&prop, dev) == hipSuccess ? prop.multiProcessorCount : 256;
    });
    if (setup[dev] != hipSuccess) return setup[dev];
    const int cus = cu_count[dev];
    int64_t slices = n / (int64_t(1) << 18);
    if (slices < 1) slices = 1;
    if (slices * passes > cus) slices = cus / passes > 0 ? cus / passes : 1;
    hipLaunchKernelGGL(tally_kernel, dim3((unsigned)slices, (unsigned)passes), dim3(TALLY_BLOCK), (size_t)bins * 2, stream,
                       unit_index, n, counters, n_counters, bins);
    return hipGetLastError();
}

hipError_t launch_fold(int32_t* replicas, int shift, int64_t n, int32_t* counters, hipStream_t stream) {
    if (n <= 0 || shift <= 0) return hipSuccess;
    const int64_t threads = (1 << shift) < 64 ? n : n * 64;
    hipLaunchKernelGGL(fold_kernel, dim3(grid_for(threads)), dim3(BLOCK), 0, stream, replicas, shift, n, counters);
    return hipGetLastError();
}

hipError_t launch_match(const ScgIndex& tab, const uint8_t* d_seqs, int32_t n, int cap, int reverse,
                        int32_t* d_index, int32_t* d_mm, hipStream_t stream) {
    if (n <= 0) return hipSuccess;
    if (tab.wide == 2) hipLaunchKernelGGL(match_kernel<Big>, dim3(grid_for(n)), dim3(BLOCK), 0, stream, tab, d_seqs, n, cap, reverse, d_index, d_mm);
    else if (tab.wide) hipLaunchKernelGGL(match_kernel<uint64_t>, dim3(grid_for(n)), dim3(BLOCK), 0, stream, tab, d_seqs, n, cap, reverse, d_index, d_mm);
    else hipLaunchKernelGGL(match_kernel<uint32_t>, dim3(grid_for(n)), dim3(BLOCK), 0, stream, tab, d_seqs, n, cap, reverse, d_index, d_mm);
    return hipGetLastError();
}

hipError_t launch_synth(const scg_synth_spec& S, char* d_out, int64_t n, hipStream_t stream) {
    if (n <= 0) return hipSuccess;
    hipLaunchKernelGGL(synth_kernel, dim3(grid_for(n)), dim3(BLOCK), 0, stream, S, d_out, n);
    return hipGetLastError();
}

}
```

screencounter_amd/csrc/scg_launch.h:

```cpp
#ifndef SCG_LAUNCH_H
#define SCG_LAUNCH_H

#include <hip/hip_runtime_api.h>

#include "../../include/scg.h"
#include "scg_common.h"

namespace scg {

bool force_general();

hipError_t launch_single(const ScgSingleParams& P, int tmpl_len, const ScgReads& R, int64_t n, const ScgCounters& counts, int32_t* flag, hipStream_t stream);
hipError_t launch_random(const ScgSingleParams& P, int tmpl_len, const ScgReads& R, int64_t n, int32_t* d_hits, int32_t* flag, hipStream_t stream);
hipError_t launch_combo(const ScgComboParams& P, int tmpl_len, const ScgReads& R, int64_t n, const ScgCounters& cells, int32_t* flag, hipStream_t stream);
hipError_t launch_dual(const ScgDualParams& P, int tmpl_len, const ScgReads& R1, const ScgReads& R2, int64_t n, const ScgCounters& counts, int32_t* flag, hipStream_t stream);
hipError_t launch_fold(int32_t* replicas, int replica_shift, int64_t n, int32_t* counters, hipStream_t stream);
hipError_t launch_hot_fold(int32_t* hot, int32_t* pair_of_counters, hipStream_t stream);
hipError_t launch_tally(const int32_t* unit_index, int64_t n, int32_t* counters, int64_t n_counters, hipStream_t stream);
size_t sort_rle_scratch_bytes(size_t n);
hipError_t launch_sort_rle(const uint64_t* d_keys, uint64_t* d_sorted, size_t n, uint64_t* d_unique, uint32_t* d_counts, uint32_t* d_runs,
                           void* d_scratch, size_t scratch_bytes, hipStream_t stream);
#define SCG_RANDOM_ROUNDS 4
struct ScgRandomTable {
    unsigned long long* tags;
    unsigned long long* counts;
    uint8_t* arena;
    unsigned long long* state;
    uint64_t mask;
    int32_t vstart, vlen;
    int32_t tag_bits;
    int32_t pad;
};
hipError_t launch_random_insert(const ScgRandomTable& T, const ScgReads& R, int64_t n, const int32_t* hits, int32_t* slots,
                                int64_t ordinal0, hipStream_t stream);
hipError_t launch_random_verify_rounds(const ScgRandomTable& T, const ScgReads& R, int64_t n, const int32_t* hits, int32_t* slots,
                                       int32_t* list_a, int32_t* list_b, int32_t* lens, hipStream_t stream);
hipError_t launch_random_rehash(const ScgRandomTable& from, const ScgRandomTable& to, hipStream_t stream);
hipError_t launch_random_compact(const ScgRandomTable& T, unsigned long long* packed_tags, unsigned long long* packed_counts,
                                 int32_t* hashed_slots, unsigned long long* hashed_counts, unsigned long long* n_out, hipStream_t stream);
size_t random_sort_scratch_bytes(size_t n);
hipError_t launch_random_sort(const unsigned long long* keys_in, unsigned long long* keys_out, const unsigned long long* vals_in,
                              unsigned long long* vals_out, size_t n, int end_bit, void* scratch, size_t scratch_bytes, hipStream_t stream);
hipError_t launch_random_decode(const unsigned long long* tags, int64_t n, int32_t vlen, char* out, hipStream_t stream);
hipError_t launch_random_gather(const ScgRandomTable& T, const int32_t* slots, int64_t n, uint8_t* out, hipStream_t stream);

hipError_t launch_match(const ScgIndex& tab, const uint8_t* d_seqs, int32_t n, int cap, int reverse,
                        int32_t* d_index, int32_t* d_mm, hipStream_t stream);
hipError_t launch_synth(const scg_synth_spec& S, char* d_out, int64_t n, hipStream_t stream);

}

#endif
```

screencounter_amd/csrc/scg_plan.cpp:

```cpp
#include "scg_internal.hpp"

namespace scgapi {
int key_class(int len) { return len > SCG_MAX_WIDE_BARCODE ? 2 : (len > SCG_MAX_BARCODE ? 1 : 0); }

scg::HostIndex build_index_class(int cls, const char* const* pool, int32_t n, int32_t len, int max_mm) {
    if (cls == 2) return scg::build_index_big(pool, n, len, max_mm);
    return cls == 1 ? scg::build_index_wide(pool, n, len, max_mm) : scg::build_index(pool, n, len, max_mm);
}
scg::HostIndex build_uid_index_class(int cls, const char* const* pool, int32_t n, int32_t len, int max_mm,
                                     std::vector<std::vector<int32_t> >& expansions, size_t& n_uid) {
    if (cls == 2) return scg::build_uid_index_big(pool, n, len, max_mm, expansions, n_uid);
    return scg::build_uid_index_wide(pool, n, len, max_mm, expansions, n_uid);
}

bool general_only(const scg_plan* P) {
    return scg::force_general() || P->tab[0].view.wide == 2 || (P->kind == scg_plan::DUAL_SE_DIAG && P->tab_combined.view.wide == 2);
}

int64_t dense_cells() {
    const char* e = getenv("SCG_DENSE_CELLS");
    if (e && *e) return std::min<int64_t>(std::max<int64_t>(atoll(e), 0), int64_t(1) << 30);
    return int64_t(1) << 26;
}

ScgReads make_reads(const char* d_seqs, const uint32_t* d_offsets, int32_t fixed_len, int32_t max_len) {
    ScgReads r;
    r.seqs = reinterpret_cast<const uint8_t*>(d_seqs);
    r.offsets = d_offsets;
    r.fixed_len = d_offsets ? 0 : fixed_len;
    r.max_len = d_offsets ? max_len : fixed_len;
#ifdef SCG_ABLATE
    const char* ab = std::getenv("SCG_ABLATE");
    r.ablate = ab ? std::atoi(ab) : 0;
#else
    r.ablate = 0;
#endif
    return r;
}

void check_reads_args(const char* d_seqs, const uint32_t* d_offsets, int32_t fixed_len, int64_t n) {
    if (n < 0) throw Error(SCG_ERR_INVALID, "negative read count");
    if (n > 0 && !d_seqs && !(d_offsets == nullptr && fixed_len == 0)) throw Error(SCG_ERR_INVALID, "null read buffer");
    if (!d_offsets && fixed_len < 0) throw Error(SCG_ERR_INVALID, "negative fixed read length");
}


std::unique_ptr<scg_plan> compile_single(const char* constant, int strand, const char* const* pool, int32_t n_pool,
                                         int mismatches, int use_first) {
    if (!constant || (n_pool > 0 && !pool) || n_pool < 0) throw Error(SCG_ERR_INVALID, "null argument");
    std::unique_ptr<scg_plan> P(new scg_plan);
    P->kind = scg_plan::SINGLE;
    int plen = scg::pool_length(pool, n_pool);
    P->ht1 = scg::parse_template(constant, strand);
    if (P->ht1.t.nreg != 1) {
        throw Error(SCG_ERR_INVALID, "expected one variable region in the constant template");
    }
    int vlen = P->ht1.t.flen[0];
    if (vlen != plen) {
        throw Error(SCG_ERR_INVALID, "length of barcode_pool sequences (" + std::to_string(plen) +
                    ") should be the same as the barcode_pool region (" + std::to_string(vlen) + ")");
    }
    if (mismatches < 0) throw Error(SCG_ERR_INVALID, "negative number of mismatches");
    P->htab[0] = plen > SCG_MAX_BARCODE ? scg::build_index_wide(pool, n_pool, plen, mismatches) : scg::build_index(pool, n_pool, plen, mismatches);
    P->scan1 = scg::build_scan(P->ht1.t, mismatches);
    P->n_pool[0] = n_pool;
    P->n_counters = n_pool;
    P->max_mm1 = mismatches;
    P->use_first = use_first != 0;
    return P;
}

std::unique_ptr<scg_plan> compile_dual_single_end(const char* constant, int strand, const char* const* const* pools, const int32_t* n_pools,
                                                  int32_t n_regions, int mismatches, int use_first) {
    if (!constant || n_regions < 0 || (n_regions > 0 && (!pools || !n_pools))) throw Error(SCG_ERR_INVALID, "null argument");
    std::unique_ptr<scg_plan> P(new scg_plan);
    P->kind = scg_plan::SINGLE;
    std::vector<int> plen(n_regions);
    for (int r = 0; r < n_regions; ++r) {
        if (n_pools[r] < 0 || (n_pools[r] > 0 && !pools[r])) throw Error(SCG_ERR_INVALID, "null argument");
        plen[r] = scg::pool_length(pools[r], n_pools[r]);
    }
    P->ht1 = scg::parse_template(constant, strand);
    const ScgTemplate& t = P->ht1.t;
    if (t.nreg != n_regions) throw Error(SCG_ERR_INVALID, "length of 'barcode_pools' should equal the number of variable regions");
    if (n_regions < 1 || n_regions > SCG_MAX_REGIONS) {
        throw Error(SCG_ERR_UNSUPPORTED, "this engine counts dual barcodes in single-end reads with 1 to " + std::to_string(SCG_MAX_REGIONS) +
                    " variable regions (got " + std::to_string(n_regions) + ")");
    }
    int total = 0;
    for (int r = 0; r < n_regions; ++r) {
        if (plen[r] != t.flen[r]) {
            throw Error(SCG_ERR_INVALID, "length of variable region " + std::to_string(r + 1) + " (" + std::to_string(t.flen[r]) +
                        ") should be the same as its sequences (" + std::to_string(plen[r]) + ")");
        }
        total += plen[r];
    }
    const int32_t n_choices = n_pools[0];
    for (int r = 1; r < n_regions; ++r) {
        if (n_pools[r] != n_choices) throw Error(SCG_ERR_INVALID, "all entries of 'barcode_pools' should have the same length");
    }
    if (mismatches < 0) throw Error(SCG_ERR_INVALID, "negative number of mismatches");
    std::vector<std::string> combined(n_choices);
    std::vector<const char*> ptrs(n_choices);
    for (int32_t c = 0; c < n_choices; ++c) {
        for (int r = 0; r < n_regions; ++r) combined[c].append(pools[r][c], plen[r]);
        ptrs[c] = combined[c].c_str();
    }
    P->htab[0] = scg::build_index_wide(ptrs.data(), n_choices, total, mismatches);
    P->scan1 = scg::build_scan(t, mismatches);
    P->n_pool[0] = n_choices;
    P->n_counters = n_choices;
    P->max_mm1 = mismatches;
    P->use_first = use_first != 0;
    return P;
}

std::unique_ptr<scg_plan> compile_combo(const char* constant, int strand,
                                        const char* const* pool0, int32_t n0, const char* const* pool1, int32_t n1,
                                        int mismatches, int use_first) {
    if (!constant || (n0 > 0 && !pool0) || (n1 > 0 && !pool1) || n0 < 0 || n1 < 0) throw Error(SCG_ERR_INVALID, "null argument");
    std::unique_ptr<scg_plan> P(new scg_plan);
    P->kind = scg_plan::COMBO;
    int len0 = scg::pool_length(pool0, n0);
    int len1 = scg::pool_length(pool1, n1);
    P->ht1 = scg::parse_template(constant, strand);
    if (P->ht1.t.nreg != 2) {
        throw Error(SCG_ERR_INVALID, "expected 2 variable regions in the constant template");
    }
    int lens[2] = {len0, len1};
    for (int r = 0; r < 2; ++r) {
        if (P->ht1.t.flen[r] != lens[r]) {
            throw Error(SCG_ERR_INVALID, "length of variable region " + std::to_string(r + 1) + " (" + std::to_string(P->ht1.t.flen[r]) +
                        ") should be the same as its sequences (" + std::to_string(lens[r]) + ")");
        }
    }
    if (mismatches < 0) throw Error(SCG_ERR_INVALID, "negative number of mismatches");
    const int cls = std::max(key_class(len0), key_class(len1));
    P->htab[0] = build_index_class(cls, pool0, n0, len0, mismatches);
    P->htab[1] = build_index_class(cls, pool1, n1, len1, mismatches);
    P->scan1 = scg::build_scan(P->ht1.t, mismatches);
    P->n_pool[0] = n0; P->n_pool[1] = n1;
    int64_t cells = static_cast<int64_t>(n0) * static_cast<int64_t>(n1);
    P->sparse = cells > dense_cells();
    P->n_counters = P->sparse ? 0 : cells;
    P->max_mm1 = mismatches;
    P->use_first = use_first != 0;
    return P;
}

std::unique_ptr<scg_plan> compile_dual(const char* constant1, int reverse1, int mismatches1, const char* const* pool1,
                                       const char* constant2, int reverse2, int mismatches2, const char* const* pool2,
                                       int32_t n_pool, int randomized, int use_first, int diagnostics) {
    if (!constant1 || !constant2 || (n_pool > 0 && (!pool1 || !pool2)) || n_pool < 0) throw Error(SCG_ERR_INVALID, "null argument");
    std::unique_ptr<scg_plan> P(new scg_plan);
    P->kind = scg_plan::DUAL;
    int len1 = scg::pool_length(pool1, n_pool);
    int len2 = scg::pool_length(pool2, n_pool);
    P->ht1 = scg::parse_template(constant1, reverse1 ? 1 : 0);
    P->ht2 = scg::parse_template(constant2, reverse2 ? 1 : 0);
    if (P->ht1.t.nreg != 1) throw Error(SCG_ERR_INVALID, "expected one variable region in the first constant template");
    if (P->ht1.t.flen[0] != len1) {
        throw Error(SCG_ERR_INVALID, "length of variable sequences (" + std::to_string(len1) + ") should be the same as the variable region (" +
                    std::to_string(P->ht1.t.flen[0]) + ")");
    }
    if (P->ht2.t.nreg != 1) throw Error(SCG_ERR_INVALID, "expected one variable region in the second constant template");
    if (P->ht2.t.flen[0] != len2) {
        throw Error(SCG_ERR_INVALID, "length of variable sequences (" + std::to_string(len2) + ") should be the same as the variable region (" +
                    std::to_string(P->ht2.t.flen[0]) + ")");
    }
    if (mismatches1 < 0 || mismatches2 < 0) throw Error(SCG_ERR_INVALID, "negative number of mismatches");
    std::vector<std::vector<int32_t> > exp1, exp2;
    std::vector<uint64_t> uk1, uk2;
    size_t n_uid1 = 0, n_uid2 = 0;
    if (const int cls = std::max(key_class(len1), key_class(len2))) {
        P->htab[0] = build_uid_index_class(cls, pool1, n_pool, len1, mismatches1, exp1, n_uid1);
        P->htab[1] = build_uid_index_class(cls, pool2, n_pool, len2, mismatches2, exp2, n_uid2);
    } else {
        P->htab[0] = scg::build_uid_index(pool1, n_pool, len1, mismatches1, exp1, uk1);
        P->htab[1] = scg::build_uid_index(pool2, n_pool, len2, mismatches2, exp2, uk2);
        n_uid1 = uk1.size(); n_uid2 = uk2.size();
    }
    P->scan1 = scg::build_scan(P->ht1.t, mismatches1);
    P->scan2 = scg::build_scan(P->ht2.t, mismatches2);
    P->hpairs = scg::build_pair_table(exp1, uk1, exp2, uk2);
    P->n_pool[0] = P->n_pool[1] = n_pool;
    P->n_counters = n_pool;
    if (diagnostics) {
        auto firsts = [&](const std::vector<std::vector<int32_t> >& exp, size_t n_uid) {
            std::vector<int32_t> f(n_uid, -1);
            for (size_t i = 0; i < exp.size(); ++i) {
                for (int32_t u : exp[i]) if (f[u] < 0) f[u] = static_cast<int32_t>(i);
            }
            return f;
        };
        P->first1 = firsts(exp1, n_uid1);
        P->first2 = firsts(exp2, n_uid2);
        int64_t cells = static_cast<int64_t>(n_uid1) * static_cast<int64_t>(n_uid2);
        P->sparse = cells > dense_cells();
        P->diagnostics = 1;
        P->n_counters = static_cast<int64_t>(n_pool) + 2 + (P->sparse ? 0 : cells);
    }
    P->max_mm1 = mismatches1; P->max_mm2 = mismatches2;
    P->rev1 = reverse1 != 0; P->rev2 = reverse2 != 0;
    P->randomized = randomized != 0;
    P->use_first = use_first != 0;
    return P;
}

std::unique_ptr<scg_plan> compile_dual_single_end_diag(const char* constant, int strand, const char* const* const* pools, const int32_t* n_pools,
                                                       int32_t n_regions, int mismatches, int use_first) {
    auto P = compile_dual_single_end(constant, strand, pools, n_pools, n_regions, mismatches, use_first);
    const ScgTemplate& t = P->ht1.t;
    if (t.nreg != 2) throw Error(SCG_ERR_INVALID, "expected 2 variable regions in the constant template");
    P->kind = scg_plan::DUAL_SE_DIAG;
    P->htab_combined = std::move(P->htab[0]);
    std::vector<std::vector<int32_t> > exp0, exp1;
    std::vector<uint64_t> uk0, uk1;
    size_t n_uid0 = 0, n_uid1 = 0;
    if (const int cls = std::max(key_class(t.flen[0]), key_class(t.flen[1]))) {
        P->htab[0] = build_uid_index_class(cls, pools[0], n_pools[0], t.flen[0], mismatches, exp0, n_uid0);
        P->htab[1] = build_uid_index_class(cls, pools[1], n_pools[1], t.flen[1], mismatches, exp1, n_uid1);
    } else {
        P->htab[0] = scg::build_uid_index(pools[0], n_pools[0], t.flen[0], mismatches, exp0, uk0);
        P->htab[1] = scg::build_uid_index(pools[1], n_pools[1], t.flen[1], mismatches, exp1, uk1);
        n_uid0 = uk0.size(); n_uid1 = uk1.size();
    }
    auto firsts = [&](const std::vector<std::vector<int32_t> >& exp, size_t n_uid) {
        std::vector<int32_t> f(n_uid, -1);
        for (size_t i = 0; i < exp.size(); ++i) {
            for (int32_t u : exp[i]) if (f[u] < 0) f[u] = static_cast<int32_t>(i);
        }
        return f;
    };
    P->first1 = firsts(exp0, n_uid0);
    P->first2 = firsts(exp1, n_uid1);
    int64_t cells = static_cast<int64_t>(n_uid0) * static_cast<int64_t>(n_uid1);
    P->sparse = cells > dense_cells();
    P->n_pool[1] = P->n_pool[0];
    P->n_counters = static_cast<int64_t>(P->n_pool[0]) + 2 + (P->sparse ? 0 : cells);
    return P;
}

std::unique_ptr<scg_plan> compile_paired_combo(const char* constant1, int reverse1, int mismatches1, const char* const* pool1, int32_t n1,
                                               const char* constant2, int reverse2, int mismatches2, const char* const* pool2, int32_t n2,
                                               int randomized, int use_first) {
    if (!constant1 || !constant2 || (n1 > 0 && !pool1) || (n2 > 0 && !pool2) || n1 < 0 || n2 < 0) throw Error(SCG_ERR_INVALID, "null argument");
    std::unique_ptr<scg_plan> P(new scg_plan);
    P->kind = scg_plan::DUAL;
    int len1 = scg::pool_length(pool1, n1);
    int len2 = scg::pool_length(pool2, n2);
    P->ht1 = scg::parse_template(constant1, reverse1 ? 1 : 0);
    P->ht2 = scg::parse_template(constant2, reverse2 ? 1 : 0);
    auto check = [](const scg::HostTemplate& ht, int plen) {
        if (ht.t.nreg != 1) throw Error(SCG_ERR_INVALID, "expected one variable region in the constant template");
        if (ht.t.flen[0] != plen) {
            throw Error(SCG_ERR_INVALID, "length of barcode_pool sequences (" + std::to_string(plen) +
                        ") should be the same as the barcode_pool region (" + std::to_string(ht.t.flen[0]) + ")");
        }
    };
    check(P->ht1, len1);
    check(P->ht2, len2);
    if (mismatches1 < 0 || mismatches2 < 0) throw Error(SCG_ERR_INVALID, "negative number of mismatches");
    const int cls = std::max(key_class(len1), key_class(len2));
    P->htab[0] = build_index_class(cls, pool1, n1, len1, mismatches1);
    P->htab[1] = build_index_class(cls, pool2, n2, len2, mismatches2);
    P->scan1 = scg::build_scan(P->ht1.t, mismatches1);
    P->scan2 = scg::build_scan(P->ht2.t, mismatches2);
    int64_t cells = static_cast<int64_t>(n1) * static_cast<int64_t>(n2);
    P->sparse = cells > dense_cells();
    P->first1.resize(n1);
    P->first2.resize(n2);
    for (int32_t i = 0; i < n1; ++i) P->first1[i] = i;
    for (int32_t i = 0; i < n2; ++i) P->first2[i] = i;
    P->n_pool[0] = P->n_pool[1] = 0;
    P->diagnostics = 2;
    P->n_counters = 2 + (P->sparse ? 0 : cells);
    P->max_mm1 = mismatches1; P->max_mm2 = mismatches2;
    P->rev1 = reverse1 != 0; P->rev2 = reverse2 != 0;
    P->randomized = randomized != 0;
    P->use_first = use_first != 0;
    return P;
}

ScgCounters plan_counters(const scg_plan* P) {
    ScgCounters c;
    if (P->replica_shift > 0) {
        c.base = P->replicas.as<int32_t>();
        c.replica_shift = static_cast<uint32_t>(P->replica_shift);
        c.replica_mask = (1u << P->replica_shift) - 1u;
    } else {
        c.base = P->counters; c.replica_mask = 0; c.replica_shift = 0;
    }
    c.unit_index = nullptr;
    c.unit_pair = nullptr;
    c.hot = P->hot.p ? P->hot.as<int32_t>() : nullptr;
    return c;
}


void retire_pairs(scg_plan* P, hipStream_t stream, scg_plan::PairStream& ps) {
    if (!ps.pending) return;
    uint32_t runs = 0;
    HIP_CHECK(hipEventSynchronize(ps.done));
    HIP_CHECK(hipMemcpy(&runs, ps.runs.p, sizeof(runs), hipMemcpyDeviceToHost));
    std::vector<uint64_t> keys(runs);
    std::vector<uint32_t> counts(runs);
    if (runs) {
        HIP_CHECK(hipMemcpy(keys.data(), ps.unique.p, sizeof(uint64_t) * runs, hipMemcpyDeviceToHost));
        HIP_CHECK(hipMemcpy(counts.data(), ps.counts.p, sizeof(uint32_t) * runs, hipMemcpyDeviceToHost));
    }
    for (uint32_t i = 0; i < runs; ++i) {
        if (keys[i] != ~uint64_t(0)) P->sparse_counts[keys[i]] += counts[i];
    }
    ps.pending = 0;
}

uint64_t* begin_pairs(scg_plan* P, hipStream_t stream, int64_t n) {
    scg_plan::PairStream& ps = P->pair_stream[stream];
    retire_pairs(P, stream, ps);
    const size_t m = static_cast<size_t>(std::max<int64_t>(n, 1));
    ps.keys.ensure(m * sizeof(uint64_t));
    ps.sorted.ensure(m * sizeof(uint64_t));
    ps.unique.ensure(m * sizeof(uint64_t));
    ps.counts.ensure(m * sizeof(uint32_t));
    if (!ps.runs.p) ps.runs.alloc(sizeof(uint32_t));
    ps.scratch.ensure(scg::sort_rle_scratch_bytes(m));
    HIP_CHECK(hipMemsetAsync(ps.keys.p, 0xFF, m * sizeof(uint64_t), stream));
    return ps.keys.as<uint64_t>();
}

void finish_pairs(scg_plan* P, hipStream_t stream, int64_t n) {
    scg_plan::PairStream& ps = P->pair_stream[stream];
    HIP_CHECK(scg::launch_sort_rle(ps.keys.as<uint64_t>(), ps.sorted.as<uint64_t>(), static_cast<size_t>(n), ps.unique.as<uint64_t>(),
                                   ps.counts.as<uint32_t>(), ps.runs.as<uint32_t>(), ps.scratch.p, ps.scratch.bytes, stream));
    if (!ps.done) HIP_CHECK(hipEventCreateWithFlags(&ps.done, hipEventDisableTiming));
    HIP_CHECK(hipEventRecord(ps.done, stream));
    ps.pending = n;
}

void retire_all_pairs(scg_plan* P) {
    DeviceGuard g(P->device);
    for (auto& kv : P->pair_stream) retire_pairs(P, kv.first, kv.second);
}

bool use_tally(const scg_plan* P, int64_t n) {
    if (P->diagnostics) return false;
    if (const char* e = std::getenv("SCG_TALLY")) { if (*e) return *e != '0'; }
    return P->n_counters >= 4096 && P->n_counters <= 4 * 80 * 1024 && n >= (int64_t(1) << 20);
}

void fold_replicas(scg_plan* P, hipStream_t stream) {
    if (P->replica_shift > 0) {
        HIP_CHECK(scg::launch_fold(P->replicas.as<int32_t>(), P->replica_shift, P->n_counters, P->counters, stream));
    }
}

void launch_batch_se_diag(scg_plan* P, const ScgReads& R, int64_t n, hipStream_t stream) {
    scg_plan::Timer timer(P, stream);
    DevBuf& buf = P->unit_index[stream];
    buf.ensure(static_cast<size_t>(n) * sizeof(int32_t));
    ScgSingleParams sp;
    sp.scan = P->scan1;
    sp.tmpl = P->d_tmpl1.as<ScgTemplate>();
    sp.index = P->tab_combined.view;
    sp.max_mm = P->max_mm1; sp.use_first = P->use_first;
    sp.fwd = P->ht1.fwd; sp.rev = P->ht1.rev;
    ScgCounters c1;
    c1.base = P->counters; c1.replica_mask = 0; c1.replica_shift = 0; c1.hot = nullptr; c1.unit_pair = nullptr;
    c1.unit_index = buf.as<int32_t>();
    HIP_CHECK(scg::launch_single(sp, P->ht1.t.len, R, n, c1, P->error_flag.as<int32_t>(), stream));
    HIP_CHECK(scg::launch_tally(c1.unit_index, n, P->counters, P->n_pool[0], stream));
    ScgComboParams cp;
    cp.scan = P->scan1;
    cp.tmpl = P->d_tmpl1.as<ScgTemplate>();
    cp.index[0] = P->tab[0].view; cp.index[1] = P->tab[1].view;
    cp.n_pool[0] = static_cast<int32_t>(P->first1.size()); cp.n_pool[1] = static_cast<int32_t>(P->first2.size());
    cp.max_mm = P->max_mm1; cp.use_first = P->use_first;
    cp.fwd = P->ht1.fwd; cp.rev = P->ht1.rev;
    cp.only_if_negative = c1.unit_index; cp.keep_first = 1; cp.pad = 0;
    ScgCounters c2;
    c2.base = P->counters + P->n_pool[0] + 2; c2.replica_mask = 0; c2.replica_shift = 0; c2.unit_index = nullptr; c2.hot = nullptr;
    c2.unit_pair = P->sparse ? begin_pairs(P, stream, n) : nullptr;
    HIP_CHECK(scg::launch_combo(cp, P->ht1.t.len, R, n, c2, P->error_flag.as<int32_t>(), stream));
    timer.stop();
    if (P->sparse) finish_pairs(P, stream, n);
    P->total += n;
}


std::unique_ptr<scg_plan> compile_random(const char* constant, int strand, int mismatches, int use_first) {
    if (!constant) throw Error(SCG_ERR_INVALID, "null argument");
    std::unique_ptr<scg_plan> P(new scg_plan);
    P->kind = scg_plan::RANDOM;
    P->ht1 = scg::parse_template(constant, strand);
    const ScgTemplate& t = P->ht1.t;
    if (t.nreg < 1) throw Error(SCG_ERR_INVALID, "expected one variable region in the constant template");
    if (t.nreg > SCG_MAX_REGIONS) throw Error(SCG_ERR_UNSUPPORTED, "this engine handles templates with at most " + std::to_string(SCG_MAX_REGIONS) + " variable regions");
    if (mismatches < 0) throw Error(SCG_ERR_INVALID, "negative number of mismatches");
    P->scan1 = scg::build_scan(t, mismatches);
    P->max_mm1 = mismatches;
    P->use_first = use_first != 0;
    P->n_counters = 0;
    P->rnd.reset(new RandomTally);
    P->rnd->vstart = t.fstart[0];
    P->rnd->vlen = t.flen[0];
    if (const char* e = std::getenv("SCG_TEST_RANDOM_TAG_BITS")) {
        if (*e) P->rnd->tag_bits = std::min(std::max(std::atoi(e), 0), 61);
    }
    return P;
}

namespace {

const uint64_t RANDOM_INITIAL_SLOTS = uint64_t(1) << 16;
const uint64_t RANDOM_MAX_SLOTS = uint64_t(1) << 30;

void swap_buf(DevBuf& a, DevBuf& b) { std::swap(a.p, b.p); std::swap(a.bytes, b.bytes); }

void alloc_table(DevBuf& tags, DevBuf& counts, DevBuf& arena, uint64_t cap, int vlen) {
    tags.alloc(cap * sizeof(unsigned long long));
    counts.alloc(cap * sizeof(unsigned long long));
    arena.alloc(cap * static_cast<uint64_t>(vlen));
}

void random_order(RandomTally& T, hipStream_t stream) {
    if (T.has_last) HIP_CHECK(hipStreamWaitEvent(stream, T.last, 0));
}
void random_done(RandomTally& T, hipStream_t stream) {
    HIP_CHECK(hipEventRecord(T.last, stream));
    T.has_last = true;
}

ScgSingleParams random_params(const scg_plan* P) {
    ScgSingleParams sp;
    sp.scan = P->scan1;
    sp.tmpl = P->d_tmpl1.as<ScgTemplate>();
    std::memset(&sp.index, 0, sizeof(sp.index));
    sp.max_mm = P->max_mm1; sp.use_first = P->use_first;
    sp.fwd = P->ht1.fwd; sp.rev = P->ht1.rev;
    return sp;
}

void random_reserve(scg_plan* P, int64_t n, hipStream_t stream) {
    RandomTally& T = *P->rnd;
    if (T.snap_pending && hipEventQuery(T.snap_event) == hipSuccess) {
        T.known_occ = static_cast<int64_t>(*T.snap.as<unsigned long long>());
        T.known_at = T.snap_at;
        T.snap_pending = false;
    }
    auto bound = [&] { return static_cast<uint64_t>(T.known_occ + (P->total - T.known_at) + n); };
    if (bound() * 2 <= T.cap) return;
    HIP_CHECK(hipMemcpyAsync(T.snap.p, T.state.as<unsigned long long>() + 1, sizeof(unsigned long long), hipMemcpyDeviceToHost, stream));
    HIP_CHECK(hipStreamSynchronize(stream));
    T.known_occ = static_cast<int64_t>(*T.snap.as<unsigned long long>());
    T.known_at = P->total;
    T.snap_pending = false;
    uint64_t cap = T.cap;
    while (bound() * 2 > cap) {
        if (cap >= RANDOM_MAX_SLOTS) {
            throw Error(SCG_ERR_UNSUPPORTED, "random barcode tally: " + std::to_string(bound()) + " possible keys exceed the table limit of " +
                        std::to_string(RANDOM_MAX_SLOTS / 2) + " (read out, reset and count the rest in another plan)");
        }
        cap *= 2;
    }
    if (cap == T.cap) return;
    DevBuf tags, counts, arena;
    try {
        alloc_table(tags, counts, arena, cap, T.vlen);
    } catch (const Error& e) {
        throw Error(SCG_ERR_DEVICE, "random barcode tally: cannot grow the table from " + std::to_string(T.cap) + " to " + std::to_string(cap) +
                    " slots (" + e.what() + "); no key was dropped, the counts so far stay readable");
    }
    HIP_CHECK(hipMemsetAsync(tags.p, 0, tags.bytes, stream));
    HIP_CHECK(hipMemsetAsync(counts.p, 0, counts.bytes, stream));
    const scg::ScgRandomTable from = T.view();
    scg::ScgRandomTable to = from;
    to.tags = tags.as<unsigned long long>(); to.counts = counts.as<unsigned long long>(); to.arena = arena.as<uint8_t>(); to.mask = cap - 1;
    HIP_CHECK(scg::launch_random_rehash(from, to, stream));
    HIP_CHECK(hipStreamSynchronize(stream));
    swap_buf(T.tags, tags); swap_buf(T.counts, counts); swap_buf(T.arena, arena);
    T.cap = cap;
}

void launch_batch_random(scg_plan* P, const ScgReads& R, int64_t n, hipStream_t stream) {
    RandomTally& T = *P->rnd;
    if (n >= INT32_MAX) throw Error(SCG_ERR_INVALID, "random-barcode plans take batches of fewer than 2^31 - 1 reads");
    random_order(T, stream);
    if (n > 0) {
        random_reserve(P, n, stream);
        RandomTally::Scratch& s = T.scratch[stream];
        const size_t bytes = static_cast<size_t>(n) * sizeof(int32_t);
        s.hits.ensure(bytes); s.slots.ensure(bytes); s.list_a.ensure(bytes); s.list_b.ensure(bytes);
        s.lens.ensure(SCG_RANDOM_ROUNDS * sizeof(int32_t));
        scg_plan::Timer timer(P, stream);
        HIP_CHECK(hipMemsetAsync(s.hits.p, 0xFF, bytes, stream));
        HIP_CHECK(hipMemsetAsync(s.lens.p, 0, SCG_RANDOM_ROUNDS * sizeof(int32_t), stream));
        HIP_CHECK(scg::launch_random(random_params(P), P->ht1.t.len, R, n, s.hits.as<int32_t>(), P->error_flag.as<int32_t>(), stream));
        const scg::ScgRandomTable view = T.view();
        HIP_CHECK(scg::launch_random_insert(view, R, n, s.hits.as<int32_t>(), s.slots.as<int32_t>(), P->total, stream));
        HIP_CHECK(scg::launch_random_verify_rounds(view, R, n, s.hits.as<int32_t>(), s.slots.as<int32_t>(), s.list_a.as<int32_t>(),
                                                   s.list_b.as<int32_t>(), s.lens.as<int32_t>(), stream));
        timer.stop();
        P->total += n;
        if (!T.snap_pending) {
            HIP_CHECK(hipMemcpyAsync(T.snap.p, T.state.as<unsigned long long>() + 1, sizeof(unsigned long long), hipMemcpyDeviceToHost, stream));
            HIP_CHECK(hipEventRecord(T.snap_event, stream));
            T.snap_pending = true;
            T.snap_at = P->total;
        }
    }
    random_done(T, stream);
}

}

void random_to_device(scg_plan* P) {
    RandomTally& T = *P->rnd;
    DeviceGuard g(P->device);
    T.cap = RANDOM_INITIAL_SLOTS;
    alloc_table(T.tags, T.counts, T.arena, T.cap, T.vlen);
    T.state.alloc(4 * sizeof(unsigned long long));
    T.snap.ensure(sizeof(unsigned long long));
    HIP_CHECK(hipEventCreateWithFlags(&T.snap_event, hipEventDisableTiming));
    HIP_CHECK(hipEventCreateWithFlags(&T.last, hipEventDisableTiming));
    HIP_CHECK(hipMemset(T.tags.p, 0, T.tags.bytes));
    HIP_CHECK(hipMemset(T.counts.p, 0, T.counts.bytes));
    HIP_CHECK(hipMemset(T.state.p, 0, T.state.bytes));
    HIP_CHECK(hipMemset(T.state.p, 0xFF, sizeof(unsigned long long)));
    HIP_CHECK(hipStreamSynchronize(nullptr));
}

void random_reset(scg_plan* P, hipStream_t stream) {
    RandomTally& T = *P->rnd;
    random_order(T, stream);
    HIP_CHECK(hipMemsetAsync(T.tags.p, 0, T.tags.bytes, stream));
    HIP_CHECK(hipMemsetAsync(T.counts.p, 0, T.counts.bytes, stream));
    HIP_CHECK(hipMemsetAsync(T.state.p, 0, T.state.bytes, stream));
    HIP_CHECK(hipMemsetAsync(T.state.p, 0xFF, sizeof(unsigned long long), stream));
    HIP_CHECK(hipMemsetAsync(P->error_flag.p, 0, sizeof(int32_t), stream));
    random_done(T, stream);
    T.known_occ = T.known_at = 0;
    T.snap_pending = false;
}

void read_random(scg_plan* P, hipStream_t stream, char** sequences_out, int32_t** freq_out, int64_t* k_out, int32_t* length_out) {
    RandomTally& T = *P->rnd;
    DeviceGuard g(P->device);
    random_order(T, stream);
    unsigned long long st[4] = {0, 0, 0, 0};
    HIP_CHECK(hipMemcpyAsync(st, T.state.p, sizeof(st), hipMemcpyDeviceToHost, stream));
    HIP_CHECK(hipStreamSynchronize(stream));
    if (st[0] != ~0ull) {
        throw Error(SCG_ERR_INVALID, std::string("cannot complement unknown base '") + static_cast<char>(st[0] & 0xFF) + "'");
    }
    read_counters(P, nullptr);
    if (st[2]) {
        throw Error(SCG_ERR_UNSUPPORTED, "random barcode tally: the keys of " + std::to_string(st[2]) + " reads collided with other keys in all " +
                    std::to_string(SCG_RANDOM_ROUNDS) + " hash rounds; counts are incomplete");
    }
    const uint64_t occ = st[1];
    const int vlen = T.vlen;
    const size_t m = static_cast<size_t>(std::max<uint64_t>(occ, 1));
    DevBuf ptags, pcounts, hslots, hcounts, nout;
    ptags.alloc(m * 8); pcounts.alloc(m * 8); hslots.alloc(m * 4); hcounts.alloc(m * 8); nout.alloc(2 * 8);
    HIP_CHECK(hipMemsetAsync(nout.p, 0, 2 * 8, stream));
    HIP_CHECK(scg::launch_random_compact(T.view(), ptags.as<unsigned long long>(), pcounts.as<unsigned long long>(), hslots.as<int32_t>(),
                                         hcounts.as<unsigned long long>(), nout.as<unsigned long long>(), stream));
    unsigned long long nn[2] = {0, 0};
    HIP_CHECK(hipMemcpyAsync(nn, nout.p, sizeof(nn), hipMemcpyDeviceToHost, stream));
    HIP_CHECK(hipStreamSynchronize(stream));
    const size_t np = static_cast<size_t>(nn[0]), nh = static_cast<size_t>(nn[1]);
    const size_t stride = static_cast<size_t>(vlen) + 1;
    std::vector<unsigned long long> pc(np), hc(nh);
    std::vector<char> pbytes(np * stride);
    std::vector<uint8_t> hbytes(nh * static_cast<size_t>(vlen));
    if (np) {
        DevBuf stags, scounts, scratch, dec;
        stags.alloc(np * 8); scounts.alloc(np * 8);
        scratch.alloc(scg::random_sort_scratch_bytes(np));
        dec.alloc(np * stride);
        HIP_CHECK(scg::launch_random_sort(ptags.as<unsigned long long>(), stags.as<unsigned long long>(), pcounts.as<unsigned long long>(),
                                          scounts.as<unsigned long long>(), np, 2 * vlen, scratch.p, scratch.bytes, stream));
        HIP_CHECK(scg::launch_random_decode(stags.as<unsigned long long>(), static_cast<int64_t>(np), vlen, dec.as<char>(), stream));
        HIP_CHECK(hipMemcpyAsync(pc.data(), scounts.p, np * 8, hipMemcpyDeviceToHost, stream));
        HIP_CHECK(hipMemcpyAsync(pbytes.data(), dec.p, np * stride, hipMemcpyDeviceToHost, stream));
        HIP_CHECK(hipStreamSynchronize(stream));
    }
    std::vector<size_t> horder(nh);
    if (nh) {
        DevBuf gathered;
        gathered.alloc(hbytes.size());
        HIP_CHECK(scg::launch_random_gather(T.view(), hslots.as<int32_t>(), static_cast<int64_t>(nh), gathered.as<uint8_t>(), stream));
        HIP_CHECK(hipMemcpyAsync(hbytes.data(), gathered.p, hbytes.size(), hipMemcpyDeviceToHost, stream));
        HIP_CHECK(hipMemcpyAsync(hc.data(), hcounts.p, nh * 8, hipMemcpyDeviceToHost, stream));
        HIP_CHECK(hipStreamSynchronize(stream));
        for (size_t i = 0; i < nh; ++i) horder[i] = i;
        const uint8_t* hb = hbytes.data();
        std::sort(horder.begin(), horder.end(), [&](size_t a, size_t b) {
            return std::memcmp(hb + a * vlen, hb + b * vlen, static_cast<size_t>(vlen)) < 0;
        });
    }
    random_done(T, stream);
    auto narrow = [](unsigned long long c) {
        if (c > static_cast<unsigned long long>(INT32_MAX)) {
            throw Error(SCG_ERR_INVALID, "frequency of a random barcode (" + std::to_string(c) + ") exceeds the 32-bit range of the count vectors");
        }
        return static_cast<int32_t>(c);
    };
    const size_t K = np + nh;
    char* so = static_cast<char*>(std::malloc(K * stride + 1));
    int32_t* fo = static_cast<int32_t*>(std::malloc(sizeof(int32_t) * (K + 1)));
    if (!so || !fo) { std::free(so); std::free(fo); throw std::bad_alloc(); }
    try {
        size_t a = 0, b = 0;
        for (size_t k = 0; k < K; ++k) {
            const bool take_packed = b == nh ||
                (a < np && std::memcmp(pbytes.data() + a * stride, hbytes.data() + horder[b] * vlen, static_cast<size_t>(vlen)) < 0);
            if (take_packed) {
                std::memcpy(so + k * stride, pbytes.data() + a * stride, stride);
                fo[k] = narrow(pc[a++]);
            } else {
                std::memcpy(so + k * stride, hbytes.data() + horder[b] * vlen, static_cast<size_t>(vlen));
                so[k * stride + vlen] = 0;
                fo[k] = narrow(hc[horder[b++]]);
            }
        }
    } catch (...) {
        std::free(so); std::free(fo);
        throw;
    }
    *sequences_out = so; *freq_out = fo; *k_out = static_cast<int64_t>(K); *length_out = vlen;
}

void launch_batch(scg_plan* P, const ScgReads& R, int64_t n, hipStream_t stream) {
    if (P->kind == scg_plan::RANDOM) { launch_batch_random(P, R, n, stream); return; }
    if (P->kind == scg_plan::DUAL_SE_DIAG) { launch_batch_se_diag(P, R, n, stream); return; }
    scg_plan::Timer timer(P, stream);
    if (P->kind == scg_plan::SINGLE) {
        ScgSingleParams sp;
        sp.scan = P->scan1;
        sp.tmpl = P->d_tmpl1.as<ScgTemplate>();
        sp.index = P->tab[0].view;
        sp.max_mm = P->max_mm1; sp.use_first = P->use_first;
        sp.fwd = P->ht1.fwd; sp.rev = P->ht1.rev;
            ScgCounters counts = plan_counters(P);
        const bool tally = use_tally(P, n) && R.max_len > 0 && R.max_len <= 320 && !general_only(P);
        if (tally) {
            DevBuf& buf = P->unit_index[stream];
            buf.ensure(static_cast<size_t>(n) * sizeof(int32_t));
            counts.unit_index = buf.as<int32_t>();
        }
        HIP_CHECK(scg::launch_single(sp, P->ht1.t.len, R, n, counts, P->error_flag.as<int32_t>(), stream));
        if (tally) {
            timer.stop();
            HIP_CHECK(scg::launch_tally(counts.unit_index, n, P->counters, P->n_counters, stream));
            P->total += n;
            return;
        }
    } else {
        ScgComboParams cp;
        cp.scan = P->scan1;
        cp.tmpl = P->d_tmpl1.as<ScgTemplate>();
        cp.index[0] = P->tab[0].view; cp.index[1] = P->tab[1].view;
        cp.n_pool[0] = P->n_pool[0]; cp.n_pool[1] = P->n_pool[1];
        cp.max_mm = P->max_mm1; cp.use_first = P->use_first;
        cp.fwd = P->ht1.fwd; cp.rev = P->ht1.rev;
        cp.only_if_negative = nullptr; cp.keep_first = 0; cp.pad = 0;
        ScgCounters counts = plan_counters(P);
        if (P->sparse) {
            counts.unit_pair = begin_pairs(P, stream, n);
            HIP_CHECK(scg::launch_combo(cp, P->ht1.t.len, R, n, counts, P->error_flag.as<int32_t>(), stream));
            timer.stop();
            finish_pairs(P, stream, n);
            P->total += n;
            return;
        }
        const bool tally = use_tally(P, n) && R.max_len > 0 && R.max_len <= 320 && !general_only(P);
        if (tally) {
            DevBuf& buf = P->unit_index[stream];
            buf.ensure(static_cast<size_t>(n) * sizeof(int32_t));
            counts.unit_index = buf.as<int32_t>();
        }
        HIP_CHECK(scg::launch_combo(cp, P->ht1.t.len, R, n, counts, P->error_flag.as<int32_t>(), stream));
        if (tally) {
            timer.stop();
            HIP_CHECK(scg::launch_tally(counts.unit_index, n, P->counters, P->n_counters, stream));
            P->total += n;
            return;
        }
    }
    timer.stop();
    fold_replicas(P, stream);
    P->total += n;
}

ScgScan searched_strand_first(const ScgScan& t, bool reverse) {
    if (!reverse) return t;
    ScgScan o = t;
    o.fseeds = t.rseeds; o.rseeds = t.fseeds;
    for (int r = 0; r < SCG_MAX_REGIONS; ++r) {
        o.fstart[r] = t.rstart[r]; o.rstart[r] = t.fstart[r];
        o.flen[r] = t.rlen[r]; o.rlen[r] = t.flen[r];
    }
    for (int w = 0; w < SCG_MAX_TEMPLATE / 32; ++w) {
        o.fplane0[w] = t.rplane0[w]; o.rplane0[w] = t.fplane0[w];
        o.fplane1[w] = t.rplane1[w]; o.rplane1[w] = t.fplane1[w];
        o.fmask[w] = t.rmask[w]; o.rmask[w] = t.fmask[w];
    }
    return o;
}

void launch_batch_paired(scg_plan* P, const ScgReads& R1, const ScgReads& R2, int64_t n, hipStream_t stream) {
    scg_plan::Timer timer(P, stream);
    ScgDualParams dp;
    dp.scan1 = searched_strand_first(P->scan1, P->rev1); dp.scan2 = searched_strand_first(P->scan2, P->rev2);
    dp.tmpl1 = P->d_tmpl1.as<ScgTemplate>(); dp.tmpl2 = P->d_tmpl2.as<ScgTemplate>();
    dp.index1 = P->tab[0].view; dp.index2 = P->tab[1].view; dp.pairs = P->pairs.view;
    dp.rev1 = P->rev1; dp.rev2 = P->rev2; dp.max_mm1 = P->max_mm1; dp.max_mm2 = P->max_mm2;
    dp.randomized = P->randomized; dp.use_first = P->use_first;
    dp.diagnostics = P->diagnostics; dp.n_pool = P->diagnostics == 2 ? 0 : P->n_pool[0]; dp.n_uid2 = static_cast<int32_t>(P->first2.size());
    dp.keep_first = P->diagnostics == 1; dp.only_if_negative = nullptr;
    ScgCounters counts = plan_counters(P);
    if (P->sparse) counts.unit_pair = begin_pairs(P, stream, n);
    const int lo_len = std::min(R1.max_len, R2.max_len), hi_len = std::max(R1.max_len, R2.max_len);
    const bool staged = lo_len > 0 && hi_len <= 320 && !general_only(P);
    const int tmpl_len = std::max(P->ht1.t.len, P->ht2.t.len);
    dp.overflow = nullptr;
    if (staged && P->diagnostics != 2 && n < INT32_MAX) {
        DevBuf& buf = P->overflow[stream];
        buf.ensure((static_cast<size_t>(n) + 1) * sizeof(int32_t));
        dp.overflow = buf.as<int32_t>();
    }
    if (P->diagnostics == 1 && staged) {
        DevBuf& buf = P->unit_index[stream];
        buf.ensure(static_cast<size_t>(n) * sizeof(int32_t));
        ScgCounters c1 = counts;
        c1.unit_index = buf.as<int32_t>();
        c1.unit_pair = nullptr;
        dp.diagnostics = 0;
        HIP_CHECK(scg::launch_dual(dp, tmpl_len, R1, R2, n, c1, P->error_flag.as<int32_t>(), stream));
        HIP_CHECK(scg::launch_tally(c1.unit_index, n, P->counters, P->n_pool[0], stream));
        dp.diagnostics = 2;
        dp.only_if_negative = c1.unit_index;
        HIP_CHECK(scg::launch_dual(dp, tmpl_len, R1, R2, n, counts, P->error_flag.as<int32_t>(), stream));
        timer.stop();
        if (P->sparse) finish_pairs(P, stream, n);
        fold_replicas(P, stream);
        HIP_CHECK(scg::launch_hot_fold(P->hot.as<int32_t>(), P->counters + P->n_pool[0], stream));
        P->total += n;
        return;
    }
    const bool tally = use_tally(P, n) && staged;
    if (tally) {
        DevBuf& buf = P->unit_index[stream];
        buf.ensure(static_cast<size_t>(n) * sizeof(int32_t));
        counts.unit_index = buf.as<int32_t>();
    }
    HIP_CHECK(scg::launch_dual(dp, tmpl_len, R1, R2, n, counts, P->error_flag.as<int32_t>(), stream));
    timer.stop();
    if (P->sparse) finish_pairs(P, stream, n);
    if (tally) HIP_CHECK(scg::launch_tally(counts.unit_index, n, P->counters, P->n_counters, stream));
    else fold_replicas(P, stream);
    if (P->hot.p) HIP_CHECK(scg::launch_hot_fold(P->hot.as<int32_t>(), P->counters + (P->diagnostics == 2 ? 0 : P->n_pool[0]), stream));
    P->total += n;
}

}
```

Before: 29260 Mreads/s.

## Compress per-read unit index stream into 16-bit low part plus ballot bit-planes

Replaces the per-read int32 unit index buffer that feeds the tally kernel with a packed form: a 16-bit low index per read plus wavefront-ballot bit-planes holding a mapped flag and any high index bits. The intent is to cut HBM write and read traffic between the matching kernels and the tally pass. The tally kernel is rewritten to decode eight reads at a time, and the diagnostic and overflow paths use the mapped-bit plane or atomic ORs. In exchange the kernels no longer return early for tail lanes so that ballots cover full wavefronts, and there is extra ballot and plane-assembly work per wavefront.

```diff
diff --git a/screencounter_amd/csrc/scg_common.h b/screencounter_amd/csrc/scg_common.h
--- a/screencounter_amd/csrc/scg_common.h
+++ b/screencounter_amd/csrc/scg_common.h
@@ -90,11 +90,25 @@
     const int32_t* list_vals;
 };
 
+struct ScgUnitStream {
+    uint16_t* low;
+    uint64_t* planes;
+    int64_t words;
+    int32_t nplanes;
+    int32_t pad;
+};
+
+static inline int32_t scg_unit_planes(int64_t n_counters) {
+    int bits = 0;
+    for (uint64_t v = n_counters > 0 ? (uint64_t)(n_counters - 1) : 0; v; v >>= 1) ++bits;
+    return 1 + (bits > 16 ? bits - 16 : 0);
+}
+
 struct ScgCounters {
     int32_t* base;
     uint32_t replica_mask;
     uint32_t replica_shift;
-    int32_t* unit_index;
+    ScgUnitStream unit;
     uint64_t* unit_pair;
     int32_t* hot;
 };
@@ -124,7 +138,7 @@
     int32_t max_mm;
     int32_t use_first;
     int32_t fwd, rev;
-    const int32_t* only_if_negative;
+    const uint64_t* only_if_unmapped;
     int32_t keep_first;
     int32_t pad;
 };
@@ -143,7 +157,7 @@
     int32_t n_pool;
     int32_t n_uid2;
     int32_t keep_first;
-    const int32_t* only_if_negative;
+    const uint64_t* only_if_unmapped;
     int32_t* overflow;
 };
 
diff --git a/screencounter_amd/csrc/scg_engine.hip.h b/screencounter_amd/csrc/scg_engine.hip.h
--- a/screencounter_amd/csrc/scg_engine.hip.h
+++ b/screencounter_amd/csrc/scg_engine.hip.h
@@ -20,6 +20,40 @@
 __device__ __forceinline__ void count_one(const ScgCounters& C, int64_t i) {
     const uint32_t gid = blockIdx.x * blockDim.x + threadIdx.x;
     atomicAdd(C.base + ((i << C.replica_shift) | (int64_t)(gid & C.replica_mask)), 1);
+}
+
+__device__ __forceinline__ void store_unit(const ScgCounters& C, int64_t r, bool has, int idx) {
+    const ScgUnitStream& U = C.unit;
+    if (has) U.low[r] = (uint16_t)idx;
+    const bool mapped = has && idx >= 0;
+    const uint64_t active = __builtin_amdgcn_ballot_w64(true);
+    const bool leader = (int)(threadIdx.x & 63u) == __ffsll((long long)active) - 1;
+    const int64_t w = r >> 6;
+    if (w >= U.words) return;
+    const uint64_t m = __builtin_amdgcn_ballot_w64(mapped);
+    if (leader) U.planes[w] = m;
+    for (int p = 1; p < U.nplanes; ++p) {
+        const uint64_t b = __builtin_amdgcn_ballot_w64(mapped && ((idx >> (15 + p)) & 1));
+        if (leader) U.planes[(int64_t)p * U.words + w] = b;
+    }
+}
+
+__device__ __forceinline__ void patch_unit(const ScgCounters& C, int64_t r, int idx) {
+    const ScgUnitStream& U = C.unit;
+    if (idx < 0) return;
+    U.low[r] = (uint16_t)idx;
+    const int64_t w = r >> 6;
+    const unsigned long long bit = 1ull << (r & 63);
+    __hip_atomic_fetch_or(reinterpret_cast<unsigned long long*>(U.planes + w), bit, __ATOMIC_RELAXED, __HIP_MEMORY_SCOPE_AGENT);
+    for (int p = 1; p < U.nplanes; ++p) {
+        if ((idx >> (15 + p)) & 1) {
+            __hip_atomic_fetch_or(reinterpret_cast<unsigned long long*>(U.planes + (int64_t)p * U.words + w), bit, __ATOMIC_RELAXED, __HIP_MEMORY_SCOPE_AGENT);
+        }
+    }
+}
+
+__device__ __forceinline__ bool unit_mapped(const uint64_t* __restrict__ plane, int64_t r) {
+    return (plane[r >> 6] >> (r & 63)) & 1u;
 }
 
 __device__ __forceinline__ void count_flagged(const ScgCounters& C, int which, int64_t i, bool flag) {
diff --git a/screencounter_amd/csrc/scg_kernels.hip b/screencounter_amd/csrc/scg_kernels.hip
--- a/screencounter_amd/csrc/scg_kernels.hip
+++ b/screencounter_amd/csrc/scg_kernels.hip
@@ -74,11 +74,15 @@
 template<class W>
 __global__ __launch_bounds__(BLOCK) void single_kernel(ScgSingleParams P, ScgReads R, int64_t n_reads,
                                                         ScgCounters counts) {
+    static_assert(BLOCK % 64 == 0, "a wavefront's reads are one plane word of the index stream (store_unit)");
     int64_t i = (int64_t)blockIdx.x * BLOCK + threadIdx.x;
-    if (i >= n_reads) return;
-    Read rd = get_read(R, i);
-    int idx = single_read<W>(P, rd);
-    if (counts.unit_index) counts.unit_index[i] = idx;
+    const bool has = i < n_reads;
+    int idx = -1;
+    if (has) {
+        Read rd = get_read(R, i);
+        idx = single_read<W>(P, rd);
+    }
+    if (counts.unit.low) store_unit(counts, i, has, idx);
     else if (idx >= 0) count_one(counts, idx);
 }
 
@@ -164,7 +168,7 @@
                                                        ScgCounters cells) {
     int64_t i = (int64_t)blockIdx.x * BLOCK + threadIdx.x;
     if (i >= n_reads) return;
-    if (P.only_if_negative && P.only_if_negative[i] >= 0) return;
+    if (P.only_if_unmapped && unit_mapped(P.only_if_unmapped, i)) return;
     Read rd = get_read(R, i);
     int best_id[SCG_COMBO_REGIONS] = {0, 0};
     const bool found = combo_read<W>(P, rd, best_id) != 0;
@@ -332,7 +336,7 @@
                                                       ScgCounters counts) {
     int64_t i = (int64_t)blockIdx.x * BLOCK + threadIdx.x;
     if (i >= n_pairs) return;
-    if (P.diagnostics == 2 && P.only_if_negative && P.only_if_negative[i] >= 0) return;
+    if (P.diagnostics == 2 && P.only_if_unmapped && unit_mapped(P.only_if_unmapped, i)) return;
     Read a = get_read(R1, i), b = get_read(R2, i);
     int idx = P.diagnostics == 2 ? -1 : dual_pair<W>(P, a, b);
     if (idx >= 0) {
@@ -395,27 +399,32 @@
     int64_t span0 = 0;
     const bool staged = (P.scan.len <= 32 * NT) && stage_reads<NW>(R, n_reads, r0, nr, tile, span0);
     __syncthreads();
-    if ((int)threadIdx.x >= nr) return;
-    Read rd = get_read(R, r0 + threadIdx.x);
-    if (!staged || rd.n > 32 * NW) {
-        *error_flag = 1;
-        return;
-    }
-    StagedRead sr;
-    sr.bit = (int)((int64_t)(rd.p - R.seqs) - span0);
-    sr.n = rd.n;
-    int idx;
+    static_assert(STAGE_BLOCK % 64 == 0, "a wavefront's reads are one plane word of the index stream (store_unit)");
+    const bool has = (int)threadIdx.x < nr;
+    int idx = -1;
+    if (has) {
+        Read rd = get_read(R, r0 + threadIdx.x);
+        if (!staged || rd.n > 32 * NW) {
+            *error_flag = 1;
+        } else {
+            StagedRead sr;
+            sr.bit = (int)((int64_t)(rd.p - R.seqs) - span0);
+            sr.n = rd.n;
 #ifdef SCG_ABLATE
-    if (R.ablate == 2) {
-        idx = (tile.p0[threadIdx.x] == 0xdeadbeefu) ? 0 : -1;
-    } else {
-        idx = single_read_staged<NW, NT, NC, W>(P, tile, strands, sr, R.ablate);
-    }
-    if (R.ablate == 3 && idx != 0x7ffffff0 && !counts.unit_index) return;
+            if (R.ablate == 2) {
+                idx = (tile.p0[threadIdx.x] == 0xdeadbeefu) ? 0 : -1;
+            } else {
+                idx = single_read_staged<NW, NT, NC, W>(P, tile, strands, sr, R.ablate);
+            }
 #else
-    idx = single_read_staged<NW, NT, NC, W>(P, tile, strands, sr);
+            idx = single_read_staged<NW, NT, NC, W>(P, tile, strands, sr);
 #endif
-    if (counts.unit_index) counts.unit_index[r0 + threadIdx.x] = idx;
+        }
+    }
+#ifdef SCG_ABLATE
+    if (R.ablate == 3 && idx != 0x7ffffff0 && !counts.unit.low) return;
+#endif
+    if (counts.unit.low) store_unit(counts, r0 + threadIdx.x, has, idx);
     else if (idx >= 0) count_one(counts, idx);
 }
 
@@ -498,15 +507,21 @@
     int64_t span0 = 0;
     const bool staged = (P.scan.len <= 32 * NT) && stage_reads<NW>(R, n_reads, r0, nr, tile, span0);
     __syncthreads();
-    if ((int)threadIdx.x >= nr) return;
-    Read rd = get_read(R, r0 + threadIdx.x);
+    const bool has = (int)threadIdx.x < nr;
     int found = 0, best = P.max_mm + 1;
     int best_id[SCG_COMBO_REGIONS] = {0, 0};
-    if (!staged || rd.n > 32 * NW) {
-        *error_flag = 1;
-        return;
-    }
-    if (!(SECOND && P.only_if_negative[r0 + threadIdx.x] >= 0)) {
+    Read rd;
+    rd.p = R.seqs; rd.n = 0;
+    bool search = has;
+    if (has) {
+        rd = get_read(R, r0 + threadIdx.x);
+        if (!staged || rd.n > 32 * NW) {
+            *error_flag = 1;
+            search = false;
+        }
+    }
+    if (SECOND && search) search = !unit_mapped(P.only_if_unmapped, r0 + threadIdx.x);
+    if (search) {
         const ScgScan& T = P.scan;
         StagedRead sr;
         sr.bit = (int)((int64_t)(rd.p - R.seqs) - span0);
@@ -537,8 +552,9 @@
             }
         }
     }
-    if (cells.unit_index) cells.unit_index[r0 + threadIdx.x] = found ? best_id[0] * P.n_pool[1] + best_id[1] : -1;
-    else if (cells.unit_pair) cells.unit_pair[r0 + threadIdx.x] = found ? (((uint64_t)(uint32_t)best_id[0] << 32) | (uint32_t)best_id[1]) : ~0ull;
+    if (cells.unit.low) { store_unit(cells, r0 + threadIdx.x, has, found ? best_id[0] * P.n_pool[1] + best_id[1] : -1); return; }
+    if (!has) return;
+    if (cells.unit_pair) cells.unit_pair[r0 + threadIdx.x] = found ? (((uint64_t)(uint32_t)best_id[0] << 32) | (uint32_t)best_id[1]) : ~0ull;
     else if (found) count_one(cells, (int64_t)best_id[0] * P.n_pool[1] + best_id[1]);
 }
 
@@ -728,7 +744,7 @@
     const int nr = (int)((n_pairs - r0) < STAGE_BLOCK ? (n_pairs - r0) : STAGE_BLOCK);
     const bool fits = P.scan1.len <= 32 * NT && P.scan2.len <= 32 * NT;
     const bool lane = (int)threadIdx.x < nr;
-    const bool wanted = lane && !(MATES_ONLY && P.only_if_negative && P.only_if_negative[r0 + threadIdx.x] >= 0);
+    const bool wanted = lane && !(MATES_ONLY && P.only_if_unmapped && unit_mapped(P.only_if_unmapped, r0 + threadIdx.x));
     PairState<W> S;
     S.bad = !fits;
     S.h1a.count = S.h2a.count = S.h1b.count = S.h2b.count = 0;
@@ -744,31 +760,34 @@
         dual_pass<NW, NT, NC, MATES_ONLY, RANDOMIZED, W>(0, P, R1, R2, n_pairs, r0, nr, fits, wanted, tile, S);
         dual_pass<NW, NT, NC, MATES_ONLY, RANDOMIZED, W>(1, P, R1, R2, n_pairs, r0, nr, fits, wanted, tile, S);
     }
-    if (!lane) return;
-    if (S.bad) { *error_flag = 1; return; }
-    if (!wanted) return;
     if (MATES_ONLY) {
+        if (!lane) return;
+        if (S.bad) { *error_flag = 1; return; }
+        if (!wanted) return;
         diagnose_pair(P, S.sm, counts);
         return;
     }
     int idx = -1;
-    if (S.h1a.count > 1 || S.h2b.count > 1 || S.h1b.count > 1 || S.h2a.count > 1) {
-        const int slot = atomicAdd(P.overflow, 1);
-        P.overflow[1 + slot] = (int32_t)(r0 + threadIdx.x);
-        if (counts.unit_index) counts.unit_index[r0 + threadIdx.x] = -1;
-        return;
-    }
-    const bool best_mode = !P.use_first;
-    int best;
-    dual_orientation_hits<W>(P, best_mode, S.h1a, S.h2b, idx, best);
-    if (RANDOMIZED && (best_mode || idx < 0)) {
-        int ci, cb;
-        dual_orientation_hits<W>(P, best_mode, S.h1b, S.h2a, ci, cb);
-        if (!best_mode) idx = ci;
-        else if (idx < 0 || best > cb) { idx = ci; best = cb; }
-        else if (best == cb && idx != ci) { idx = -1; }
-    }
-    if (counts.unit_index) counts.unit_index[r0 + threadIdx.x] = idx;
+    if (lane) {
+        if (S.bad) {
+            *error_flag = 1;
+        } else if (S.h1a.count > 1 || S.h2b.count > 1 || S.h1b.count > 1 || S.h2a.count > 1) {
+            const int slot = atomicAdd(P.overflow, 1);
+            P.overflow[1 + slot] = (int32_t)(r0 + threadIdx.x);
+        } else {
+            const bool best_mode = !P.use_first;
+            int best;
+            dual_orientation_hits<W>(P, best_mode, S.h1a, S.h2b, idx, best);
+            if (RANDOMIZED && (best_mode || idx < 0)) {
+                int ci, cb;
+                dual_orientation_hits<W>(P, best_mode, S.h1b, S.h2a, ci, cb);
+                if (!best_mode) idx = ci;
+                else if (idx < 0 || best > cb) { idx = ci; best = cb; }
+                else if (best == cb && idx != ci) { idx = -1; }
+            }
+        }
+    }
+    if (counts.unit.low) store_unit(counts, r0 + threadIdx.x, lane, idx);
     else if (idx >= 0) count_one(counts, idx);
 }
 
@@ -779,7 +798,7 @@
         const int64_t i = P.overflow[1 + k];
         Read a = get_read(R1, i), b = get_read(R2, i);
         const int idx = dual_pair<W>(P, a, b);
-        if (counts.unit_index) counts.unit_index[i] = idx;
+        if (counts.unit.low) patch_unit(counts, i, idx);
         else if (idx >= 0) count_one(counts, idx);
     }
 }
@@ -796,35 +815,42 @@
     const bool ok1 = fits && stage_reads<NW>(R1, n_pairs, r0, nr, tile1, span1);
     const bool ok2 = ok1 && stage_reads<NW>(R2, n_pairs, r0, nr, tile2, span2);
     __syncthreads();
-    if ((int)threadIdx.x >= nr) return;
-    Read a = get_read(R1, r0 + threadIdx.x), b = get_read(R2, r0 + threadIdx.x);
-    if (!ok2 || a.n > 32 * NW || b.n > 32 * NW) {
-        *error_flag = 1;
-        return;
-    }
-    StagedRead sa, sb;
-    sa.bit = (int)((int64_t)(a.p - R1.seqs) - span1); sa.n = a.n;
-    sb.bit = (int)((int64_t)(b.p - R2.seqs) - span2); sb.n = b.n;
-    const bool best_mode = !P.use_first;
-    const int norient = P.randomized ? 2 : 1;
+    const bool has = (int)threadIdx.x < nr;
     int best = 0, idx = -1;
-    for (int o = 0; o < norient; ++o) {
-        const Tile<NW>* ta = o ? &tile2 : &tile1;
-        const Tile<NW>* tb = o ? &tile1 : &tile2;
-        const StagedRead ra = o ? sb : sa, rb = o ? sa : sb;
-        int ci, cb;
-        dual_orientation_staged<NW, NT, NC, W>(P, best_mode, *ta, ra, *tb, rb, ci, cb);
-        if (!best_mode) {
-            idx = ci;
-            if (ci >= 0) break;
-        } else if (o == 0) {
-            idx = ci; best = cb;
-        } else {
-            if (idx < 0 || best > cb) { idx = ci; best = cb; }
-            else if (best == cb && idx != ci) { idx = -1; }
-        }
-    }
-    if (counts.unit_index) counts.unit_index[r0 + threadIdx.x] = idx;
+    bool search = has;
+    Read a, b;
+    a.p = R1.seqs; a.n = 0; b.p = R2.seqs; b.n = 0;
+    if (has) {
+        a = get_read(R1, r0 + threadIdx.x); b = get_read(R2, r0 + threadIdx.x);
+        if (!ok2 || a.n > 32 * NW || b.n > 32 * NW) {
+            *error_flag = 1;
+            search = false;
+        }
+    }
+    if (search) {
+        StagedRead sa, sb;
+        sa.bit = (int)((int64_t)(a.p - R1.seqs) - span1); sa.n = a.n;
+        sb.bit = (int)((int64_t)(b.p - R2.seqs) - span2); sb.n = b.n;
+        const bool best_mode = !P.use_first;
+        const int norient = P.randomized ? 2 : 1;
+        for (int o = 0; o < norient; ++o) {
+            const Tile<NW>* ta = o ? &tile2 : &tile1;
+            const Tile<NW>* tb = o ? &tile1 : &tile2;
+            const StagedRead ra = o ? sb : sa, rb = o ? sa : sb;
+            int ci, cb;
+            dual_orientation_staged<NW, NT, NC, W>(P, best_mode, *ta, ra, *tb, rb, ci, cb);
+            if (!best_mode) {
+                idx = ci;
+                if (ci >= 0) break;
+            } else if (o == 0) {
+                idx = ci; best = cb;
+            } else {
+                if (idx < 0 || best > cb) { idx = ci; best = cb; }
+                else if (best == cb && idx != ci) { idx = -1; }
+            }
+        }
+    }
+    if (counts.unit.low) store_unit(counts, r0 + threadIdx.x, has, idx);
     else if (idx >= 0) count_one(counts, idx);
 }
 
@@ -951,7 +977,7 @@
 template<int NW, int NT> struct LaunchCombo {
     template<int NC, class W>
     static void run(const ScgComboParams& P, const ScgReads& R, int64_t n, const ScgCounters& cells, int32_t* flag, hipStream_t stream) {
-        if (P.only_if_negative) hipLaunchKernelGGL((combo_staged_kernel<NW, NT, NC, true, W>), dim3(staged_grid(n)), dim3(STAGE_BLOCK), extra_lds(), stream, P, R, n, cells, flag);
+        if (P.only_if_unmapped) hipLaunchKernelGGL((combo_staged_kernel<NW, NT, NC, true, W>), dim3(staged_grid(n)), dim3(STAGE_BLOCK), extra_lds(), stream, P, R, n, cells, flag);
         else hipLaunchKernelGGL((combo_staged_kernel<NW, NT, NC, false, W>), dim3(staged_grid(n)), dim3(STAGE_BLOCK), extra_lds(), stream, P, R, n, cells, flag);
     }
     static hipError_t go(const ScgComboParams& P, const ScgReads& R, int64_t n, const ScgCounters& cells, int32_t* flag, hipStream_t stream) {
@@ -1072,17 +1098,18 @@
 
 constexpr int TALLY_BLOCK = 1024;
 
-__global__ __launch_bounds__(TALLY_BLOCK) void tally_kernel(const int32_t* __restrict__ unit_index, int64_t n, int32_t* __restrict__ counters,
+template<int H>
+__global__ __launch_bounds__(TALLY_BLOCK) void tally_kernel(ScgUnitStream S, int64_t n, int32_t* __restrict__ counters,
                                                             int64_t n_counters, int bins) {
     extern __shared__ uint32_t tally_bins[];
     const int64_t lo = (int64_t)blockIdx.y * bins;
     const int nb = (int)((n_counters - lo) < bins ? (n_counters - lo) : bins);
     for (int i = threadIdx.x; i < (bins + 1) / 2; i += TALLY_BLOCK) tally_bins[i] = 0;
     __syncthreads();
-    const int64_t quads = (n + 3) / 4;
-    const int64_t q0 = quads * blockIdx.x / gridDim.x, q1 = quads * (blockIdx.x + 1) / gridDim.x;
-    auto add = [&](int32_t v) {
-        const uint32_t b = (uint32_t)(v - (int32_t)lo);
+    const int64_t octs = (n + 7) / 8;
+    const int64_t o0 = octs * blockIdx.x / gridDim.x, o1 = octs * (blockIdx.x + 1) / gridDim.x;
+    auto add = [&](uint32_t v) {
+        const uint32_t b = v - (uint32_t)lo;
         if (b >= (uint32_t)nb) return;
         const uint32_t sh = (b & 1u) * 16u;
         const uint32_t old = atomicAdd(&tally_bins[b >> 1], 1u << sh);
@@ -1091,24 +1118,65 @@
             atomicAdd(&counters[lo + b], 0x8000);
         }
     };
-    typedef int32_t i32x4 __attribute__((ext_vector_type(4)));
-    const i32x4* quad = reinterpret_cast<const i32x4*>(unit_index);
-    const int64_t q_full = n / 4;
-    constexpr int U = 4;
-    int64_t q = q0 + threadIdx.x;
-    for (; q + (U - 1) * TALLY_BLOCK < q1 && q + (U - 1) * TALLY_BLOCK < q_full; q += U * TALLY_BLOCK) {
-        i32x4 v[U];
+    typedef uint32_t u32x4 __attribute__((ext_vector_type(4)));
+    const u32x4* low8 = reinterpret_cast<const u32x4*>(S.low);
+    const uint8_t* plane_bytes = reinterpret_cast<const uint8_t*>(S.planes);
+    const int64_t plane_stride = S.words * 8;
+    auto oct = [&](const u32x4& v, uint32_t unmapped, auto high) {
 #pragma unroll
-        for (int k = 0; k < U; ++k) v[k] = __builtin_nontemporal_load(quad + q + k * TALLY_BLOCK);
+        for (int j = 0; j < 8; ++j) {
+            const uint32_t w = j < 2 ? v.x : j < 4 ? v.y : j < 6 ? v.z : v.w;
+            add(((j & 1) ? w >> 16 : w & 0xFFFFu) | high(j) | (((unmapped >> j) & 1u) << 31));
+        }
+    };
+    if constexpr (H >= 0) {
+        constexpr int U = 4;
+        constexpr int HN = H > 0 ? H : 1;
+        int64_t o = o0 + threadIdx.x;
+        for (; o + (U - 1) * TALLY_BLOCK < o1; o += U * TALLY_BLOCK) {
+            u32x4 v[U];
+            uint32_t mb[U], hb[U][HN];
 #pragma unroll
-        for (int k = 0; k < U; ++k) { add(v[k].x); add(v[k].y); add(v[k].z); add(v[k].w); }
-    }
-    for (; q < q1; q += TALLY_BLOCK) {
-        if (q < q_full) {
-            const i32x4 v = __builtin_nontemporal_load(quad + q);
-            add(v.x); add(v.y); add(v.z); add(v.w);
-        } else {
-            for (int64_t i = 4 * q; i < n; ++i) add(unit_index[i]);
+            for (int k = 0; k < U; ++k) {
+                v[k] = __builtin_nontemporal_load(low8 + o + k * TALLY_BLOCK);
+                mb[k] = __builtin_nontemporal_load(plane_bytes + o + k * TALLY_BLOCK);
+#pragma unroll
+                for (int p = 0; p < H; ++p) hb[k][p] = __builtin_nontemporal_load(plane_bytes + (p + 1) * plane_stride + o + k * TALLY_BLOCK);
+            }
+#pragma unroll
+            for (int k = 0; k < U; ++k) {
+                oct(v[k], ~mb[k], [&](int j) {
+                    uint32_t h = 0;
+#pragma unroll
+                    for (int p = 0; p < H; ++p) h |= ((hb[k][p] >> j) & 1u) << (16 + p);
+                    return h;
+                });
+            }
+        }
+        for (; o < o1; o += TALLY_BLOCK) {
+            const u32x4 v = __builtin_nontemporal_load(low8 + o);
+            const uint32_t mb = __builtin_nontemporal_load(plane_bytes + o);
+            uint32_t hb[HN];
+#pragma unroll
+            for (int p = 0; p < H; ++p) hb[p] = __builtin_nontemporal_load(plane_bytes + (p + 1) * plane_stride + o);
+            oct(v, ~mb, [&](int j) {
+                uint32_t h = 0;
+#pragma unroll
+                for (int p = 0; p < H; ++p) h |= ((hb[p] >> j) & 1u) << (16 + p);
+                return h;
+            });
+        }
+    } else {
+        for (int64_t o = o0 + threadIdx.x; o < o1; o += TALLY_BLOCK) {
+            const u32x4 v = __builtin_nontemporal_load(low8 + o);
+            const uint32_t mb = __builtin_nontemporal_load(plane_bytes + o);
+            uint32_t hi[8] = {0, 0, 0, 0, 0, 0, 0, 0};
+            for (int p = 1; p < S.nplanes; ++p) {
+                const uint32_t hb = plane_bytes[p * plane_stride + o];
+#pragma unroll
+                for (int j = 0; j < 8; ++j) hi[j] |= ((hb >> j) & 1u) << (15 + p);
+            }
+            oct(v, ~mb, [&](int j) { return hi[j]; });
         }
     }
     __syncthreads();
@@ -1168,12 +1236,14 @@
     return hipGetLastError();
 }
 
-hipError_t launch_tally(const int32_t* unit_index, int64_t n, int32_t* counters, int64_t n_counters, hipStream_t stream) {
+hipError_t launch_tally(const ScgUnitStream& S, int64_t n, int32_t* counters, int64_t n_counters, hipStream_t stream) {
     if (n <= 0 || n_counters <= 0) return hipSuccess;
     const int max_bins = 80 * 1024;
     const int passes = (int)((n_counters + max_bins - 1) / max_bins);
     int bins = (int)((n_counters + passes - 1) / passes);
     bins = (bins + 1) & ~1;
+    typedef void (*Kernel)(ScgUnitStream, int64_t, int32_t*, int64_t, int);
+    static const Kernel kernels[5] = {tally_kernel<0>, tally_kernel<1>, tally_kernel<2>, tally_kernel<3>, tally_kernel<-1>};
     constexpr int MAX_DEVICES = 64;
     static std::once_flag once[MAX_DEVICES];
     static int cu_count[MAX_DEVICES];
@@ -1181,7 +1251,11 @@
     int dev = 0;
     if (hipGetDevice(&dev) != hipSuccess || dev < 0 || dev >= MAX_DEVICES) return hipErrorInvalidDevice;
     std::call_once(once[dev], [dev] {
-        setup[dev] = hipFuncSetAttribute(reinterpret_cast<const void*>(tally_kernel), hipFuncAttributeMaxDynamicSharedMemorySize, 80 * 1024 * 2);
+        setup[dev] = hipSuccess;
+        for (Kernel k : kernels) {
+            const hipError_t e = hipFuncSetAttribute(reinterpret_cast<const void*>(k), hipFuncAttributeMaxDynamicSharedMemorySize, 80 * 1024 * 2);
+            if (e != hipSuccess) setup[dev] = e;
+        }
         hipDeviceProp_t prop;
         cu_count[dev] = hipGetDeviceProperties(&prop, dev) == hipSuccess ? prop.multiProcessorCount : 256;
     });
@@ -1190,8 +1264,9 @@
     int64_t slices = n / (int64_t(1) << 18);
     if (slices < 1) slices = 1;
     if (slices * passes > cus) slices = cus / passes > 0 ? cus / passes : 1;
-    hipLaunchKernelGGL(tally_kernel, dim3((unsigned)slices, (unsigned)passes), dim3(TALLY_BLOCK), (size_t)bins * 2, stream,
-                       unit_index, n, counters, n_counters, bins);
+    const int high = S.nplanes - 1;
+    hipLaunchKernelGGL(kernels[high >= 0 && high <= 3 ? high : 4], dim3((unsigned)slices, (unsigned)passes), dim3(TALLY_BLOCK), (size_t)bins * 2, stream,
+                       S, n, counters, n_counters, bins);
     return hipGetLastError();
 }
 
diff --git a/screencounter_amd/csrc/scg_launch.h b/screencounter_amd/csrc/scg_launch.h
--- a/screencounter_amd/csrc/scg_launch.h
+++ b/screencounter_amd/csrc/scg_launch.h
@@ -16,7 +16,7 @@
 hipError_t launch_dual(const ScgDualParams& P, int tmpl_len, const ScgReads& R1, const ScgReads& R2, int64_t n, const ScgCounters& counts, int32_t* flag, hipStream_t stream);
 hipError_t launch_fold(int32_t* replicas, int replica_shift, int64_t n, int32_t* counters, hipStream_t stream);
 hipError_t launch_hot_fold(int32_t* hot, int32_t* pair_of_counters, hipStream_t stream);
-hipError_t launch_tally(const int32_t* unit_index, int64_t n, int32_t* counters, int64_t n_counters, hipStream_t stream);
+hipError_t launch_tally(const ScgUnitStream& S, int64_t n, int32_t* counters, int64_t n_counters, hipStream_t stream);
 size_t sort_rle_scratch_bytes(size_t n);
 hipError_t launch_sort_rle(const uint64_t* d_keys, uint64_t* d_sorted, size_t n, uint64_t* d_unique, uint32_t* d_counts, uint32_t* d_runs,
                            void* d_scratch, size_t scratch_bytes, hipStream_t stream);
diff --git a/screencounter_amd/csrc/scg_plan.cpp b/screencounter_amd/csrc/scg_plan.cpp
--- a/screencounter_amd/csrc/scg_plan.cpp
+++ b/screencounter_amd/csrc/scg_plan.cpp
@@ -291,7 +291,7 @@
     } else {
         c.base = P->counters; c.replica_mask = 0; c.replica_shift = 0;
     }
-    c.unit_index = nullptr;
+    c.unit = ScgUnitStream{nullptr, nullptr, 0, 0, 0};
     c.unit_pair = nullptr;
     c.hot = P->hot.p ? P->hot.as<int32_t>() : nullptr;
     return c;
@@ -343,6 +343,19 @@
     for (auto& kv : P->pair_stream) retire_pairs(P, kv.first, kv.second);
 }
 
+ScgUnitStream unit_stream(scg_plan* P, hipStream_t stream, int64_t n, int64_t n_counters) {
+    DevBuf& buf = P->unit_index[stream];
+    ScgUnitStream U;
+    U.words = (n + 63) / 64;
+    U.nplanes = scg_unit_planes(n_counters);
+    U.pad = 0;
+    const size_t low_bytes = static_cast<size_t>((n + 7) / 8) * 16;
+    buf.ensure(low_bytes + static_cast<size_t>(U.nplanes) * static_cast<size_t>(U.words) * sizeof(uint64_t));
+    U.low = buf.as<uint16_t>();
+    U.planes = reinterpret_cast<uint64_t*>(buf.as<char>() + low_bytes);
+    return U;
+}
+
 bool use_tally(const scg_plan* P, int64_t n) {
     if (P->diagnostics) return false;
     if (const char* e = std::getenv("SCG_TALLY")) { if (*e) return *e != '0'; }
@@ -357,8 +370,6 @@
 
 void launch_batch_se_diag(scg_plan* P, const ScgReads& R, int64_t n, hipStream_t stream) {
     scg_plan::Timer timer(P, stream);
-    DevBuf& buf = P->unit_index[stream];
-    buf.ensure(static_cast<size_t>(n) * sizeof(int32_t));
     ScgSingleParams sp;
     sp.scan = P->scan1;
     sp.tmpl = P->d_tmpl1.as<ScgTemplate>();
@@ -367,9 +378,9 @@
     sp.fwd = P->ht1.fwd; sp.rev = P->ht1.rev;
     ScgCounters c1;
     c1.base = P->counters; c1.replica_mask = 0; c1.replica_shift = 0; c1.hot = nullptr; c1.unit_pair = nullptr;
-    c1.unit_index = buf.as<int32_t>();
+    c1.unit = unit_stream(P, stream, n, P->n_pool[0]);
     HIP_CHECK(scg::launch_single(sp, P->ht1.t.len, R, n, c1, P->error_flag.as<int32_t>(), stream));
-    HIP_CHECK(scg::launch_tally(c1.unit_index, n, P->counters, P->n_pool[0], stream));
+    HIP_CHECK(scg::launch_tally(c1.unit, n, P->counters, P->n_pool[0], stream));
     ScgComboParams cp;
     cp.scan = P->scan1;
     cp.tmpl = P->d_tmpl1.as<ScgTemplate>();
@@ -377,9 +388,9 @@
     cp.n_pool[0] = static_cast<int32_t>(P->first1.size()); cp.n_pool[1] = static_cast<int32_t>(P->first2.size());
     cp.max_mm = P->max_mm1; cp.use_first = P->use_first;
     cp.fwd = P->ht1.fwd; cp.rev = P->ht1.rev;
-    cp.only_if_negative = c1.unit_index; cp.keep_first = 1; cp.pad = 0;
+    cp.only_if_unmapped = c1.unit.planes; cp.keep_first = 1; cp.pad = 0;
     ScgCounters c2;
-    c2.base = P->counters + P->n_pool[0] + 2; c2.replica_mask = 0; c2.replica_shift = 0; c2.unit_index = nullptr; c2.hot = nullptr;
+    c2.base = P->counters + P->n_pool[0] + 2; c2.replica_mask = 0; c2.replica_shift = 0; c2.unit = ScgUnitStream{nullptr, nullptr, 0, 0, 0}; c2.hot = nullptr;
     c2.unit_pair = P->sparse ? begin_pairs(P, stream, n) : nullptr;
     HIP_CHECK(scg::launch_combo(cp, P->ht1.t.len, R, n, c2, P->error_flag.as<int32_t>(), stream));
     timer.stop();
@@ -645,15 +656,11 @@
         sp.fwd = P->ht1.fwd; sp.rev = P->ht1.rev;
             ScgCounters counts = plan_counters(P);
         const bool tally = use_tally(P, n) && R.max_len > 0 && R.max_len <= 320 && !general_only(P);
-        if (tally) {
-            DevBuf& buf = P->unit_index[stream];
-            buf.ensure(static_cast<size_t>(n) * sizeof(int32_t));
-            counts.unit_index = buf.as<int32_t>();
-        }
+        if (tally) counts.unit = unit_stream(P, stream, n, P->n_counters);
         HIP_CHECK(scg::launch_single(sp, P->ht1.t.len, R, n, counts, P->error_flag.as<int32_t>(), stream));
         if (tally) {
             timer.stop();
-            HIP_CHECK(scg::launch_tally(counts.unit_index, n, P->counters, P->n_counters, stream));
+            HIP_CHECK(scg::launch_tally(counts.unit, n, P->counters, P->n_counters, stream));
             P->total += n;
             return;
         }
@@ -665,7 +672,7 @@
         cp.n_pool[0] = P->n_pool[0]; cp.n_pool[1] = P->n_pool[1];
         cp.max_mm = P->max_mm1; cp.use_first = P->use_first;
         cp.fwd = P->ht1.fwd; cp.rev = P->ht1.rev;
-        cp.only_if_negative = nullptr; cp.keep_first = 0; cp.pad = 0;
+        cp.only_if_unmapped = nullptr; cp.keep_first = 0; cp.pad = 0;
         ScgCounters counts = plan_counters(P);
         if (P->sparse) {
             counts.unit_pair = begin_pairs(P, stream, n);
@@ -676,15 +683,11 @@
             return;
         }
         const bool tally = use_tally(P, n) && R.max_len > 0 && R.max_len <= 320 && !general_only(P);
-        if (tally) {
-            DevBuf& buf = P->unit_index[stream];
-            buf.ensure(static_cast<size_t>(n) * sizeof(int32_t));
-            counts.unit_index = buf.as<int32_t>();
-        }
+        if (tally) counts.unit = unit_stream(P, stream, n, P->n_counters);
         HIP_CHECK(scg::launch_combo(cp, P->ht1.t.len, R, n, counts, P->error_flag.as<int32_t>(), stream));
         if (tally) {
             timer.stop();
-            HIP_CHECK(scg::launch_tally(counts.unit_index, n, P->counters, P->n_counters, stream));
+            HIP_CHECK(scg::launch_tally(counts.unit, n, P->counters, P->n_counters, stream));
             P->total += n;
             return;
         }
@@ -719,7 +722,7 @@
     dp.rev1 = P->rev1; dp.rev2 = P->rev2; dp.max_mm1 = P->max_mm1; dp.max_mm2 = P->max_mm2;
     dp.randomized = P->randomized; dp.use_first = P->use_first;
     dp.diagnostics = P->diagnostics; dp.n_pool = P->diagnostics == 2 ? 0 : P->n_pool[0]; dp.n_uid2 = static_cast<int32_t>(P->first2.size());
-    dp.keep_first = P->diagnostics == 1; dp.only_if_negative = nullptr;
+    dp.keep_first = P->diagnostics == 1; dp.only_if_unmapped = nullptr;
     ScgCounters counts = plan_counters(P);
     if (P->sparse) counts.unit_pair = begin_pairs(P, stream, n);
     const int lo_len = std::min(R1.max_len, R2.max_len), hi_len = std::max(R1.max_len, R2.max_len);
@@ -732,16 +735,14 @@
         dp.overflow = buf.as<int32_t>();
     }
     if (P->diagnostics == 1 && staged) {
-        DevBuf& buf = P->unit_index[stream];
-        buf.ensure(static_cast<size_t>(n) * sizeof(int32_t));
         ScgCounters c1 = counts;
-        c1.unit_index = buf.as<int32_t>();
+        c1.unit = unit_stream(P, stream, n, P->n_pool[0]);
         c1.unit_pair = nullptr;
         dp.diagnostics = 0;
         HIP_CHECK(scg::launch_dual(dp, tmpl_len, R1, R2, n, c1, P->error_flag.as<int32_t>(), stream));
-        HIP_CHECK(scg::launch_tally(c1.unit_index, n, P->counters, P->n_pool[0], stream));
+        HIP_CHECK(scg::launch_tally(c1.unit, n, P->counters, P->n_pool[0], stream));
         dp.diagnostics = 2;
-        dp.only_if_negative = c1.unit_index;
+        dp.only_if_unmapped = c1.unit.planes;
         HIP_CHECK(scg::launch_dual(dp, tmpl_len, R1, R2, n, counts, P->error_flag.as<int32_t>(), stream));
         timer.stop();
         if (P->sparse) finish_pairs(P, stream, n);
@@ -751,15 +752,11 @@
         return;
     }
     const bool tally = use_tally(P, n) && staged;
-    if (tally) {
-        DevBuf& buf = P->unit_index[stream];
-        buf.ensure(static_cast<size_t>(n) * sizeof(int32_t));
-        counts.unit_index = buf.as<int32_t>();
-    }
+    if (tally) counts.unit = unit_stream(P, stream, n, P->n_counters);
     HIP_CHECK(scg::launch_dual(dp, tmpl_len, R1, R2, n, counts, P->error_flag.as<int32_t>(), stream));
     timer.stop();
     if (P->sparse) finish_pairs(P, stream, n);
-    if (tally) HIP_CHECK(scg::launch_tally(counts.unit_index, n, P->counters, P->n_counters, stream));
+    if (tally) HIP_CHECK(scg::launch_tally(counts.unit, n, P->counters, P->n_counters, stream));
     else fold_replicas(P, stream);
     if (P->hot.p) HIP_CHECK(scg::launch_hot_fold(P->hot.as<int32_t>(), P->counters + (P->diagnostics == 2 ? 0 : P->n_pool[0]), stream));
     P->total += n;
```

New measurement: 28560 Mreads/s. -2.4%, worse.
